# CODEJIN/Glow_TTS

Hardware: AMD Instinct MI355X
Metric: mel-frames/sec (train fwd+bwd) (higher is better)
Workload: dtype bf16; 1 GPU; BASELINE config 2: Vanilla single-speaker, LJSpeech-shaped synthetic (80-mel, 800 frames, 120 tokens), batch=32/GPU, fixed Set F, Train_Step = forward+losses+backward+clip_grad_norm+RAdam+Noam schedule; mode=Vanilla, global_batch=32, mel_frames=800, parallelism=dp1

## Files before the change

glow_tts_amd/abi.py:

```python
import ctypes
from ctypes import POINTER, c_char_p

ABI_VERSION = 7
OK, E_ARG, E_LAUNCH = 0, -1, -2
F32, BF16 = 0, 1
PERM_NONE, PERM_PAIR = 0, 1
APRO_NONE, APRO_PAIRMUL, APRO_SQNEG = 0, 1, 2
EPI_LINEAR, EPI_GATE, EPI_RESSKIP, EPI_COUPLE, EPI_DGATE = 0, 1, 2, 3, 4
F_BIAS, F_RELU, F_ADD_IN0, F_MASK, F_ACCUM, F_FIRST, F_LAST, F_REVERSE, F_COLMASK, F_DROPOUT = 1, 2, 4, 8, 16, 32, 64, 128, 256, 512
F_COND_ROWS, F_GATE_IN0, F_COND_FX = 1024, 2048, 4096
IO_A_BF16, IO_IN0_BF16, IO_OUT0_BF16 = 1, 2, 4
WIO_DY_BF16, WIO_X_BF16, WIO_WIDE, WIO_DMA = 1, 2, 4, 8
ROW_PAD = 2
MAX_WN_LAYERS = 8
WN_SLAB_BYTES = 24576
WN_FUSED_MAX_LAYERS = 4
PREP_MAX_JOBS = 22
WN_BWD_MAX_JOBS = 8
SUM_MAX_SEGS = 12
C2D_MAX_LAYERS = 8
SAMPLE_SCAN_CHUNK = 1024
SAMPLE_TILE = 64
GE2E_MAX_MEL, GE2E_MAX_H, GE2E_MAX_STACKS, GE2E_MAX_E = 512, 768, 8, 1024

I, L, F, U, P = ctypes.c_int, ctypes.c_int64, ctypes.c_float, ctypes.c_uint32, ctypes.c_void_p
PI, PL = POINTER(I), POINTER(L)


def _fields(*groups):
    return [(name, t) for names, t in groups for name in names.split()]


class Packed(ctypes.Structure):
    c_name = "glowtts_packed"
    _fields_ = _fields(("w", P), ("npad kchunks", I))


class FlowDims(ctypes.Structure):
    c_name = "glowtts_flow_dims"
    _fields_ = _fields(("B T C H L ksize precision", I), ("drop_p", F), ("seed", U), ("seed_ptr", P), ("act_bf16", I))


class FlowParams(ctypes.Structure):
    c_name = "glowtts_flow_params"
    _fields_ = _fields(("an_logs an_bias winfo", P),
                       ("start", Packed), ("in_ rs", Packed * MAX_WN_LAYERS), ("end", Packed),
                       ("start_t", Packed), ("in_t rs_t", Packed * MAX_WN_LAYERS), ("end_t", Packed),
                       ("b_start", P), ("b_in b_rs", P * MAX_WN_LAYERS), ("b_end", P),
                       ("cond", P), ("ldcond", L), ("cond_rows", I), ("wn_img wn_img_t", P))


class FlowActs(ctypes.Structure):
    c_name = "glowtts_flow_acts"
    _fields_ = _fields(("xin xmid xout", P), ("hs gates", P * MAX_WN_LAYERS), ("skip outs rowmask", P), ("acts", P * MAX_WN_LAYERS),
                       ("skip_bf xa_bf next_an_logs next_an_bias next_winfo next_xmid next_xout next_xa_bf", P), ("actnorm_done", I))


class FlowGrads(ctypes.Structure):
    c_name = "glowtts_flow_grads"
    _fields_ = _fields(("dx dlogdet douts dskip", P), ("dh dins", P * MAX_WN_LAYERS), ("defer_wgrad", I),
                       ("scratch d_an dw_start db_start", P), ("dw_in db_in dw_rs db_rs", P * MAX_WN_LAYERS),
                       ("dw_end db_end dcond douts_bf", P), ("coupling_done", I), ("prev_xmid prev_outs prev_douts prev_douts_bf pitch_rows", P),
                       ("pitch_ns dh0_bf16", I))


class WnBwdJob(ctypes.Structure):
    c_name = "glowtts_wn_bwd_job"
    _fields_ = _fields(("dw v g inv_norm dv dg", P), ("rows", L), ("cols reserved", I))


class SumSeg(ctypes.Structure):
    c_name = "glowtts_sum_seg"
    _fields_ = _fields(("dst", P), ("off n", L))


class WgradJob(ctypes.Structure):
    c_name = "glowtts_wgrad_job"
    _fields_ = _fields(("dy x xmask dw dbias", P), ("lddy ldx", L), ("m ca xpro perm perm_h tile0 mt nt rows reserved", I))


class PrepJob(ctypes.Structure):
    c_name = "glowtts_prep_job"
    _fields_ = _fields(("v g inv_out packed", P), ("outer_stride inner_stride w_stride g_stride", L),
                       ("batch inner O I taps transpose perm perm_h o_ext npad kchunks tiles block0 reserved", I),
                       ("twin", P), ("twin_outer twin_inner twin_half", L), ("twin_batch twin_npad", I))


class ConvArgs(ctypes.Structure):
    c_name = "glowtts_conv_args"
    _fields_ = _fields(("a", P), ("lda", L), ("a2", P), ("lda2", L), ("ca1 ca apro rows", I), ("w", P),
                       ("n npad kchunks taps pad precision epi flags h rows_per_utt", I), ("bias rowmask cond", P), ("ldcond", L),
                       ("out0", P), ("ld0", L), ("out1", P), ("ld1", L), ("in0", P), ("ldi0", L), ("batch", I),
                       ("a_bstride w_bstride bias_bstride out_bstride mask_bstride", L), ("ncols_valid", P),
                       ("seed", U), ("drop_p", F), ("seed_ptr", P), ("io_flags", I))


class WgradArgs(ctypes.Structure):
    c_name = "glowtts_wgrad_args"
    _fields_ = _fields(("dy", P), ("lddy", L), ("x", P), ("ldx", L), ("xpro", I), ("xmask", P),
                       ("rows m ca taps pad perm perm_h precision splits accumulate", I), ("dw dbias", P), ("io_flags", I))


class PackJob(ctypes.Structure):
    c_name = "glowtts_pack_job"
    _fields_ = _fields(("w packed", P), ("O I taps transpose perm perm_h N K npad kchunks block0 reserved", I))


class OptJob(ctypes.Structure):
    c_name = "glowtts_opt_job"
    _fields_ = _fields(("p g m v", P), ("n block0", L))


class C2dPackJob(ctypes.Structure):
    c_name = "glowtts_c2d_pack_job"
    _fields_ = _fields(("w img", P), ("Ci Co cls N K npad kchunks block0", I))


class C2dReduceJob(ctypes.Structure):
    c_name = "glowtts_c2d_reduce_job"
    _fields_ = _fields(("partial dw", P), ("splits Ci Co block0", I))


SIGNATURES = {
    "glowtts_abi_version": (I, []),
    "glowtts_device_arch": (I, [c_char_p, I]),
    "glowtts_launch_count": (L, [c_char_p]),
    "glowtts_launch_log_reset": (None, []),
    "glowtts_launch_log_dump": (I, [c_char_p, I]),
    "glowtts_mfma_clock_probe": (I, [P, I, I, PI, P]),
    "glowtts_debug_stamp": (I, [P, P]),
    "glowtts_step_seed": (I, [P] * 3),
    "glowtts_mas_dp_f32": (I, [P] * 5 + [I] * 3 + [F, P]),
    "glowtts_mas_dp_f32_t": (I, [P] * 5 + [I] * 3 + [F, P]),
    "glowtts_mas_path_from_idx": (I, [P, P] + [I] * 4 + [P]),
    "glowtts_mas_f32": (I, [P] * 5 + [I] * 3 + [F, P]),
    "glowtts_mas_f32_host": (I, [P] * 4 + [I] * 3 + [F, I]),
    "glowtts_pack_weight": (I, [P] + [I] * 7 + [P, PI, PI, P]),
    "glowtts_pack_job_init": (I, [POINTER(PackJob), P] + [I] * 7 + [P, I, PI, PL]),
    "glowtts_pack_weight_multi": (I, [P] + [I] * 3 + [P]),
    "glowtts_pack_weight_batched": (I, [P] + [I] * 8 + [P, PI, PI, P]),
    "glowtts_pack_weight_strided": (I, [P] + [I] * 9 + [P] + [L] * 3 + [P]),
    "glowtts_prep_jobs_twin_in": (I, [P, PI, PI]),
    "glowtts_prep_job_init": (I, [P] * 4 + [I] * 8 + [P] + [L] * 4 + [I, PI]),
    "glowtts_prep_launch": (I, [P] + [I] * 3 + [P]),
    "glowtts_prep_launch_dev": (I, [P] + [I] * 3 + [P]),
    "glowtts_conv_chain": (I, [P] * 3),
    "glowtts_conv_cl": (I, [P, P]),
    "glowtts_squeeze_rows": (I, [P] * 4 + [I] * 4 + [P]),
    "glowtts_unsqueeze_rows": (I, [P] * 3 + [I] * 5 + [F, P]),
    "glowtts_inv1x1_prepare": (I, [P, P, I, P]),
    "glowtts_actnorm_inv1x1": (I, [P] * 6 + [L, I, I, P]),
    "glowtts_actnorm_inv1x1_pass_bf": (I, [P] * 8 + [L, I, P]),
    "glowtts_actnorm_inv1x1_pass": (I, [P] * 7 + [L, I, P]),
    "glowtts_actnorm_stats": (I, [P] * 4 + [L, I, P]),
    "glowtts_actnorm_stats_scratch_floats": (L, [L, I]),
    "glowtts_actnorm_from_stats": (I, [P] * 3 + [I, P]),
    "glowtts_coupling_bwd": (I, [P] * 6 + [L] + [I] * 3 + [P]),
    "glowtts_coupling_bwd_bf16": (I, [P] * 7 + [L] + [I] * 3 + [P]),
    "glowtts_fill_zero": (I, [P, L, P]),
    "glowtts_actnorm_inv1x1_bwd": (I, [P] * 9 + [L, I, P]),
    "glowtts_actnorm_bwd_blocks": (L, [L]),
    "glowtts_actnorm_inv1x1_bwd_coupling": (I, [P] * 8 + [L, I] + [P] * 5 + [I, I, P]),
    "glowtts_colsum_batched": (I, [P, P] + [I] * 3 + [L, L, P]),
    "glowtts_decoder_param_grads": (I, [P] * 7 + [I] * 4 + [P]),
    "glowtts_decoder_logdet": (I, [P, L] + [P] * 5 + [I] * 5 + [P]),
    "glowtts_wgrad_cl": (I, [P, P]),
    "glowtts_wgrad_grouped": (I, [P] + [I] * 9 + [P]),
    "glowtts_wgrad_grouped_io": (I, [P] + [I] * 10 + [P]),
    "glowtts_wgrad_grouped_phased": (I, [P] + [I] * 5 + [P]),
    "glowtts_flow_forward": (I, [P] * 4),
    "glowtts_flow_inverse": (I, [P] * 4),
    "glowtts_flow_encode": (I, [P] * 4),
    "glowtts_flow_backward": (I, [P] * 5),
    "glowtts_wavenet_image_bytes": (I, [I, I, PL]),
    "glowtts_wavenet_pack_images": (I, [P] * 5 + [I] * 3 + [P] * 3),
    "glowtts_wavenet_prep_jobs": (I, [P, I, PI, PI] + [P] * 13 + [I] * 3 + [P, I, P]),
    "glowtts_wavenet_fwd": (I, [P] * 5 + [I, I, P]),
    "glowtts_wavenet_bwd": (I, [P] * 5),
    "glowtts_wavenet_debug_safe_waits": (None, [I]),
    "glowtts_utt_colsum": (I, [P, L, P, L] + [I] * 5 + [P]),
    "glowtts_cond_linear_fwd": (I, [P] * 6 + [I] * 4 + [P]),
    "glowtts_cond_linear_bwd_scratch_floats": (L, [I] * 3),
    "glowtts_cond_linear_supported": (I, [I] * 3),
    "glowtts_fx_to_float": (I, [P, P, L, P]),
    "glowtts_cond_linear_bwd": (I, [P, L] + [P] * 9 + [I] * 3 + [P]),
    "glowtts_gru_fwd": (I, [P] * 5 + [I] * 3 + [P]),
    "glowtts_gru_bwd": (I, [P] * 6 + [I] * 3 + [P]),
    "glowtts_gst_supported": (I, [I] * 7),
    "glowtts_gst_keep_floats": (L, [I] * 6),
    "glowtts_gst_fwd": (I, [P, P, I] + [P] * 13 + [I] * 7 + [P]),
    "glowtts_gst_bwd": (I, [P] * 3 + [I] + [P] * 18 + [I] * 7 + [P]),
    "glowtts_conv3x3s2_supported": (I, [I] * 5),
    "glowtts_conv3x3s2_image_bytes": (I, [I] * 3 + [PL, PL]),
    "glowtts_conv3x3s2_pack_job_init": (I, [POINTER(C2dPackJob), P] + [I] * 4 + [P, I, PI]),
    "glowtts_conv3x3s2_pack": (I, [P] + [I] * 3 + [P]),
    "glowtts_conv3x3s2_fwd": (I, [P] * 4 + [I] * 7 + [P]),
    "glowtts_conv3x3s2_dgrad": (I, [P, POINTER(P), P, P] + [I] * 6 + [P]),
    "glowtts_conv3x3s2_wgrad_scratch_floats": (L, [I] * 5),
    "glowtts_conv3x3s2_wgrad": (I, [P] * 3 + [I] * 6 + [PI, P]),
    "glowtts_conv3x3s2_wgrad_reduce": (I, [POINTER(C2dReduceJob), I, P]),
    "glowtts_layernorm_fwd": (I, [P] * 8 + [L, I, F, I, F, U, P, P]),
    "glowtts_layernorm_fwd_io": (I, [P] * 8 + [L, I, F, I, F, U] + [P] * 3),
    "glowtts_proj_layernorm": (I, [P, L, P, I] + [P] * 10 + [L, I, F, F, U, P, P]),
    "glowtts_layernorm_qkv": (I, [P] * 10 + [I, P, P, L, I, F, P]),
    "glowtts_layernorm_scratch_floats": (L, [L, I]),
    "glowtts_layernorm_bwd": (I, [P] * 9 + [L, I, I, F, P]),
    "glowtts_layernorm_bwd_io": (I, [P] * 9 + [L, I, I, F, P, P, F, P]),
    "glowtts_gate_bwd": (I, [P] * 4 + [L, I, F, P]),
    "glowtts_gate_bwd_io": (I, [P] * 4 + [L, I, F, I, P]),
    "glowtts_token_masks": (I, [P] * 3 + [I, I, P]),
    "glowtts_embedding_fwd": (I, [P] * 4 + [I] * 3 + [F, P]),
    "glowtts_embedding_bwd": (I, [P] * 4 + [I] * 4 + [F, P]),
    "glowtts_rpr_attention_fwd": (I, [P] * 6 + [I] * 5 + [F, U, P, P]),
    "glowtts_rpr_attention_scratch_floats": (L, [I] * 5),
    "glowtts_rpr_attention_bwd": (I, [P] * 11 + [I] * 5 + [F, U, P, P]),
    "glowtts_rpr_attention_fwd_prec": (I, [P] * 6 + [I] * 5 + [F, U, P, I, P]),
    "glowtts_rpr_attention_bwd_partial_rows": (L, [I] * 5),
    "glowtts_rpr_attention_fwd_eval": (I, [P] * 5 + [I] * 6 + [P]),
    "glowtts_rpr_attention_bwd_prec": (I, [P] * 11 + [I] * 5 + [F, U, P, I, P]),
    "glowtts_logprior_prep": (I, [P] * 9 + [I] * 5 + [PI, PI, P]),
    "glowtts_expand_fwd": (I, [P] * 3 + [I] * 4 + [P]),
    "glowtts_expand_bwd": (I, [P] * 3 + [I] * 4 + [P]),
    "glowtts_duration_targets": (I, [P] * 3 + [I] * 3 + [P]),
    "glowtts_mle_loss_fwd": (I, [P] * 8 + [L] + [I] * 3 + [P]),
    "glowtts_mle_loss_bwd": (I, [P] * 8 + [L, P, I, P]),
    "glowtts_expand_pair_targets": (I, [P] * 8 + [I] * 4 + [P]),
    "glowtts_prior_loss_bwd": (I, [P] * 10 + [I] * 4 + [P]),
    "glowtts_mse_loss_fwd": (I, [P] * 3 + [L, F, P, I] + [P] * 3),
    "glowtts_mse_loss_bwd": (I, [P] * 4 + [L, F, P, I, P, P]),
    "glowtts_prior_loss": (I, [P] * 17 + [I] * 6 + [P]),
    "glowtts_dur_proj_supported": (I, [I]),
    "glowtts_dur_proj_fwd": (I, [P] * 5 + [I] * 4 + [P]),
    "glowtts_dur_proj_bwd": (I, [P] * 9 + [I] * 4 + [P]),
    "glowtts_prior_split_fwd": (I, [P] * 3 + [I] * 4 + [P]),
    "glowtts_prior_split_bwd": (I, [P] * 3 + [I] * 4 + [P]),
    "glowtts_weightnorm_fwd": (I, [P] * 4 + [L, I, P]),
    "glowtts_weightnorm_bwd": (I, [P] * 6 + [L, I, P]),
    "glowtts_weightnorm_bwd_multi": (I, [P, I, P]),
    "glowtts_opt_chunk": (I, []),
    "glowtts_multi_grad_norm": (I, [P, I, I, F] + [P] * 3),
    "glowtts_sum_slices": (I, [P, P, I, L, P]),
    "glowtts_sum_slices_seg": (I, [P, I, L, P, I, P]),
    "glowtts_multi_grad_scale": (I, [P, I, I, P, P]),
    "glowtts_radam_step": (I, [P, I, I] + [P] * 3),
    "glowtts_vocoder_supported": (I, [I] * 3),
    "glowtts_mel_to_linear_f32": (I, [P] * 4 + [I] * 4 + [F, P]),
    "glowtts_stft_f32": (I, [P] * 5 + [I] * 6 + [P]),
    "glowtts_istft_f32": (I, [P] * 6 + [I] * 6 + [P]),
    "glowtts_overlap_add_f32": (I, [P] * 4 + [I] * 6 + [P]),
    "glowtts_griffin_lim_step_f32": (I, [P] * 6 + [F, P] + [I] * 6 + [P]),
    "glowtts_mel_analysis_f32": (I, [P] * 7 + [I] * 8 + [F] * 3 + [P]),
    "glowtts_yin_f32": (I, [P] * 4 + [I] * 7 + [F, F, P]),
    "glowtts_prior_sample": (I, [P] * 9 + [I] * 4 + [P]),
    "glowtts_pwg_supported": (I, [I] * 5),
    "glowtts_pwg_condition": (I, [P] * 5 + [I] + [P] * 2 + [I] * 4 + [P]),
    "glowtts_pwg_first": (I, [P] * 6 + [I] * 4 + [P]),
    "glowtts_pwg_layer": (I, [P] * 9 + [I] * 8 + [P]),
    "glowtts_pwg_head": (I, [P] * 7 + [I] * 4 + [F, P]),
    "glowtts_ge2e_supported": (I, [I] * 4),
    "glowtts_ge2e_image_floats": (L, [I] * 3),
    "glowtts_ge2e_work_floats": (L, [L] + [I] * 3),
    "glowtts_ge2e_pack": (I, [P] * 6 + [I] * 4 + [P]),
    "glowtts_ge2e_forward": (I, [P] * 9 + [I] * 7 + [P]),
    "glowtts_ge2e_train_image_floats": (L, [I] * 2),
    "glowtts_ge2e_train_keep_floats": (L, [L] + [I] * 3),
    "glowtts_ge2e_train_loss_work_floats": (L, [L] + [I] * 2),
    "glowtts_ge2e_train_work_floats": (L, [L] + [I] * 4),
    "glowtts_ge2e_train_pack": (I, [P] * 3 + [I] * 3 + [P]),
    "glowtts_ge2e_train_forward": (I, [P] * 7 + [I] * 6 + [P]),
    "glowtts_ge2e_train_loss": (I, [P] * 6 + [I] * 3 + [P]),
    "glowtts_ge2e_train_backward": (I, [P] * 8 + [I] * 5 + [P]),
    "glowtts_ge2e_train_wgrad": (I, [P] * 8 + [I] * 6 + [P]),
}
```

glow_tts_amd/csrc/actnorm_math.h:

```cpp
#pragma once
__device__ __forceinline__ void actnorm_mix4(const float (&x)[4], const float (&e)[4], const float (&b)[4], const float (&w)[16], float m, float (&o)[4])
{
    float v[4];
#pragma unroll
    for (int k = 0; k < 4; ++k) v[k] = __builtin_fmaf(e[k], x[k], b[k]) * m;
#pragma unroll
    for (int k = 0; k < 4; ++k)
        o[k] = __builtin_fmaf(w[k * 4 + 3], v[3], __builtin_fmaf(w[k * 4 + 2], v[2], __builtin_fmaf(w[k * 4 + 1], v[1], w[k * 4 + 0] * v[0]))) * m;
}
```

glow_tts_amd/csrc/flow.hip:

```cpp
#include <hip/hip_runtime.h>
#include <stdint.h>
#include <string.h>
#include <stdlib.h>
#include "../../include/glowtts_hip.h"
#include "tunable.h"

namespace {

#define CHECK(x) do { int rc_ = (x); if (rc_ != GLOWTTS_OK) return rc_; } while (0)

struct Ctx {
    const glowtts_flow_dims* d; const glowtts_flow_params* p; const glowtts_flow_acts* a; void* s;
    int Tp, R, C2, H, pad;
};

Ctx make_ctx(const glowtts_flow_dims* d, const glowtts_flow_params* p, const glowtts_flow_acts* a, void* s) {
    Ctx c{d, p, a, s, 0, 0, 0, 0, 0};
    c.Tp = d->T + 2 * GLOWTTS_ROW_PAD; c.R = d->B * c.Tp; c.C2 = d->C / 2; c.H = d->H; c.pad = (d->ksize - 1) / 2;
    return c;
}

int check_dims(const glowtts_flow_dims* d) {
    if (!d || d->B < 1 || d->T < 1 || d->C < 4 || (d->C & 3) || d->H < 1 || (d->H & 3) || d->L < 1 || d->L > GLOWTTS_MAX_WN_LAYERS) return GLOWTTS_E_ARG;
    if (d->ksize != 1 && d->ksize != 3 && d->ksize != 5) return GLOWTTS_E_ARG;
// ... 35 lines not shown
            a.out0 = g; a.ld0 = 2 * H; a.io_flags = bf ? (GLOWTTS_IO_A_BF16 | GLOWTTS_IO_OUT0_BF16) : 0;
            if (acts) { a.out1 = acts; a.ld1 = H; }
            CHECK(glowtts_conv_cl(&a, c.s));
        }
        const bool last = (l == L - 1);
        glowtts_conv_args rs = base_args(c, p->rs[l], 1);
        {
            glowtts_conv_args& a = rs;
            if (acts) { a.a = acts; a.lda = H; a.ca = H; }
            else      { a.a = g; a.lda = 2 * H; a.ca = H; a.apro = GLOWTTS_APRO_PAIRMUL; }
            a.n = last ? H : 2 * H; a.h = H;
            a.epi = GLOWTTS_EPI_RESSKIP; a.flags = (l == 0 ? GLOWTTS_F_FIRST : 0) | (last ? GLOWTTS_F_LAST : 0);
            a.bias = p->b_rs[l];
            a.in0 = hin; a.ldi0 = H; a.out0 = last ? A->skip : hout; a.ld0 = H; a.out1 = A->skip; a.ld1 = H;
            a.io_flags = bf ? (GLOWTTS_IO_A_BF16 | GLOWTTS_IO_IN0_BF16 | GLOWTTS_IO_OUT0_BF16) : 0;
            if (bf && last && A->skip_bf) { a.out0 = A->skip_bf; a.ld0 = H; }
        }
        if (!last) { CHECK(glowtts_conv_cl(&rs, c.s)); continue; }
        glowtts_conv_args a = base_args(c, p->end, 1);
        if (bf && A->skip_bf) { a.a = A->skip_bf; a.io_flags = GLOWTTS_IO_A_BF16; } else a.a = A->skip;
        a.lda = H; a.ca = H; a.n = c.d->C; a.h = c.C2;
        a.epi = GLOWTTS_EPI_COUPLE; a.flags = reverse ? GLOWTTS_F_REVERSE : 0; a.bias = p->b_end;
        a.in0 = xsrc + c.C2; a.ldi0 = c.d->C;
        a.out0 = xdst + c.C2; a.ld0 = c.d->C;
        a.out1 = keep ? A->outs : nullptr; a.ld1 = p->end.npad;
        const bool chain = GLOWTTS_TUNABLE("GLOWTTS_CHAIN", 1) != 0;
        if (chain && bf && acts && A->skip_bf && glowtts_conv_chain(&rs, &a, c.s) == GLOWTTS_OK) continue;
        CHECK(glowtts_conv_cl(&rs, c.s));
        CHECK(glowtts_conv_cl(&a, c.s));
    }
    return GLOWTTS_OK;
}

__global__ void copy_half_kernel(const float* __restrict__ src, float* __restrict__ dst, long rows, int C, int n)
{
    const int q = n / 4;
    const long total = rows * q;
    for (long i = blockIdx.x * 256L + threadIdx.x; i < total; i += (long)gridDim.x * 256) {
        const long r = i / q; const int c = (int)(i - r * q) * 4;
        *reinterpret_cast<float4*>(dst + r * C + c) = *reinterpret_cast<const float4*>(src + r * C + c);
    }
}
int copy_half(const float* src, float* dst, long rows, int C, int n, void* s) {
    if (src == dst) return GLOWTTS_OK;
    if (n & 3) return GLOWTTS_E_ARG;
    long g = (rows * (n / 4) + 255) / 256; if (g > 2048) g = 2048;
    hipLaunchKernelGGL(copy_half_kernel, dim3((int)g), dim3(256), 0, static_cast<hipStream_t>(s), src, dst, rows, C, n);
    return hipGetLastError() == hipSuccess ? GLOWTTS_OK : GLOWTTS_E_LAUNCH;
}

template <typename XT>
__global__ __launch_bounds__(256) void utt_colsum_kernel(const XT* __restrict__ x, long ldx, float* __restrict__ out, long ldout,
                                                         int rows_per_utt, int n, int perm, int perm_h)
{
    const int b = blockIdx.y;
    const int col = blockIdx.x * 256 + threadIdx.x;
    if (col >= n) return;
    int pc = col;
    if (perm == GLOWTTS_PERM_PAIR) { const int hs = col / perm_h, j = col - hs * perm_h; pc = (j >> 5) * 64 + hs * 32 + (j & 31); }
    const XT* xb = x + (long)b * rows_per_utt * ldx + pc;
    float s = 0.f;
    for (int r = 0; r < rows_per_utt; ++r) s += (float)xb[(long)r * ldx];
    out[(long)b * ldout + col] = s;
}

int utt_colsum(const float* x, int64_t ldx, float* out, int64_t ldout, int B, int rows_per_utt, int n, int perm, int perm_h, bool x_bf16, void* stream)
{
    if (!x || !out || B < 1 || rows_per_utt < 1 || n < 1) return GLOWTTS_E_ARG;
    const dim3 grid((n + 255) / 256, B);
    hipStream_t s = static_cast<hipStream_t>(stream);
    if (x_bf16) hipLaunchKernelGGL(utt_colsum_kernel<__bf16>, grid, dim3(256), 0, s, reinterpret_cast<const __bf16*>(x), (long)ldx, out, (long)ldout, rows_per_utt, n, perm, perm_h);
    else hipLaunchKernelGGL(utt_colsum_kernel<float>, grid, dim3(256), 0, s, x, (long)ldx, out, (long)ldout, rows_per_utt, n, perm, perm_h);
    return hipGetLastError() == hipSuccess ? GLOWTTS_OK : GLOWTTS_E_LAUNCH;
}

}

extern "C" int glowtts_utt_colsum(const float* x, int64_t ldx, float* out, int64_t ldout, int B, int rows_per_utt, int n,
                                  int perm, int perm_h, void* stream)
{
    return utt_colsum(x, ldx, out, ldout, B, rows_per_utt, n, perm, perm_h, false, stream);
}

extern "C" int glowtts_flow_forward(const glowtts_flow_dims* d, const glowtts_flow_params* p, const glowtts_flow_acts* a, void* stream)
{
    CHECK(check_dims(d));
    if (!p || !a || !a->xin || !a->xmid || !a->xout || !a->rowmask || !a->outs) return GLOWTTS_E_ARG;
    if (!a->skip && !(p->wn_img && a->skip_bf)) return GLOWTTS_E_ARG;
    if (d->act_bf16) for (int l = 0; l < d->L; ++l) if (!a->acts[l]) return GLOWTTS_E_ARG;
    const Ctx c = make_ctx(d, p, a, stream);
    if (a->next_xmid && (!p->wn_img || !a->next_an_logs || !a->next_an_bias || !a->next_winfo || !a->next_xout)) return GLOWTTS_E_ARG;
    if (!a->actnorm_done)
        CHECK(glowtts_actnorm_inv1x1_pass_bf(a->xin, a->xmid, a->xout, a->xa_bf, p->an_logs, p->an_bias, p->winfo, a->rowmask, c.R, d->C, stream));
    return coupling_net(c, a->xmid, a->xout, false, true);
}

extern "C" int glowtts_flow_encode(const glowtts_flow_dims* d, const glowtts_flow_params* p, const glowtts_flow_acts* a, void* stream)
{
    CHECK(check_dims(d));
    if (d->drop_p != 0.f) return GLOWTTS_E_ARG;
    if (!p || !a || !a->xin || !a->xmid || !a->xout || !a->rowmask) return GLOWTTS_E_ARG;
    if (!p->wn_img) {
        if (!a->skip || !a->hs[0] || !a->hs[1] || !a->gates[0]) return GLOWTTS_E_ARG;
        if (d->act_bf16 && !a->acts[0]) return GLOWTTS_E_ARG;
    }
    if (a->next_xmid) {
        if (!p->wn_img || !a->next_an_logs || !a->next_an_bias || !a->next_winfo || !a->next_xout) return GLOWTTS_E_ARG;
        if (a->next_xmid == a->xmid || a->next_xout == a->xmid || a->xout == a->xmid || a->next_xmid == a->xout) return GLOWTTS_E_ARG;
    }
    const Ctx c = make_ctx(d, p, a, stream);
    if (!a->actnorm_done)
        CHECK(glowtts_actnorm_inv1x1_pass_bf(a->xin, a->xmid, a->xout, a->xa_bf, p->an_logs, p->an_bias, p->winfo, a->rowmask, c.R, d->C, stream));
    return coupling_net(c, a->xmid, a->xout, false, false);
}

extern "C" int glowtts_flow_inverse(const glowtts_flow_dims* d, const glowtts_flow_params* p, const glowtts_flow_acts* a, void* stream)
{
    CHECK(check_dims(d));
    if (!p || !a || !a->xin || !a->xmid || !a->xout || !a->rowmask) return GLOWTTS_E_ARG;
    if (!p->wn_img) {
        if (!a->skip || !a->hs[0] || !a->hs[1] || !a->gates[0]) return GLOWTTS_E_ARG;
        if (d->act_bf16 && !a->acts[0]) return GLOWTTS_E_ARG;
    }
    const Ctx c = make_ctx(d, p, a, stream);
    CHECK(copy_half(a->xout, a->xmid, c.R, d->C, c.C2, stream));
    CHECK(coupling_net(c, a->xout, a->xmid, true, false));
    return glowtts_actnorm_inv1x1(a->xmid, a->xin, p->an_logs, p->an_bias, p->winfo, a->rowmask, c.R, d->C, 1, stream);
}

extern "C" int glowtts_flow_backward(const glowtts_flow_dims* d, const glowtts_flow_params* p, const glowtts_flow_acts* a,
                                     const glowtts_flow_grads* g, void* stream)
{
    CHECK(check_dims(d));
    if (!p || !a || !g || !g->dx || !g->dlogdet || !g->dskip || !g->dh[0] || !g->dins[0] || !g->scratch) return GLOWTTS_E_ARG;
    const Ctx c = make_ctx(d, p, a, stream);
    const int H = c.H, L = d->L, C = d->C, C2 = c.C2, R = c.R;
    const int ldo = p->end.npad;
    const int ldin = p->in[0].npad;
    auto wargs = [&](const float* dy, int lddy, int m, const float* x, int ldx, int ca, int taps, float* dw, float* db) {
        glowtts_wgrad_args w; memset(&w, 0, sizeof(w));
        w.dy = dy; w.lddy = lddy; w.m = m; w.x = x; w.ldx = ldx; w.ca = ca; w.rows = R; w.taps = taps; w.pad = (taps - 1) / 2;
        w.precision = d->precision; w.splits = 0; w.accumulate = 1; w.dw = dw; w.dbias = db;
        return w;
    };

    const bool bf = d->act_bf16 != 0;
    const bool bfg = bf;
    const bool dbf = bfg && g->douts_bf != nullptr;
    if (!g->douts && (!dbf || !g->defer_wgrad)) return GLOWTTS_E_ARG;
    if (g->coupling_done) {  }
    else if (dbf) CHECK(glowtts_coupling_bwd_bf16(g->dx, a->xmid, a->outs, g->douts, g->douts_bf, a->rowmask, g->dlogdet, R, C, ldo, c.Tp, stream));
    else     CHECK(glowtts_coupling_bwd(g->dx, a->xmid, a->outs, g->douts, a->rowmask, g->dlogdet, R, C, ldo, c.Tp, stream));
    if (p->wn_img_t) {
        CHECK(glowtts_wavenet_bwd(d, p, a, g, stream));
        if (g->prev_outs && g->d_an) return GLOWTTS_E_ARG;
        if (g->prev_outs)
            return glowtts_actnorm_inv1x1_bwd_coupling(g->dx, g->dx, a->xin, p->an_logs, p->an_bias, p->winfo, a->rowmask, g->scratch, R, C,
                                                       g->prev_xmid, g->prev_outs, g->prev_douts, g->prev_douts_bf, g->dlogdet, ldo, c.Tp, stream);
        return glowtts_actnorm_inv1x1_bwd(g->dx, g->dx, a->xin, p->an_logs, p->an_bias, p->winfo, a->rowmask, g->d_an, g->scratch, R, C, stream);
    }
    glowtts_conv_args endq = base_args(c, p->end_t, 1);
    endq.a = dbf ? g->douts_bf : g->douts; endq.lda = ldo; endq.ca = ldo; endq.n = H; endq.epi = GLOWTTS_EPI_LINEAR; endq.flags = GLOWTTS_F_MASK;
    endq.out0 = g->dskip; endq.ld0 = H; endq.io_flags = (dbf ? GLOWTTS_IO_A_BF16 : 0) | (bfg ? GLOWTTS_IO_OUT0_BF16 : 0);
    bool end_done = false;
    if (!g->defer_wgrad) {
        glowtts_wgrad_args w = wargs(g->douts, ldo, ldo, a->skip, H, H, 1, g->dw_end, g->db_end);
        w.perm = GLOWTTS_PERM_PAIR; w.perm_h = C2;
        CHECK(glowtts_wgrad_cl(&w, stream));
    }
    const bool wg = !g->defer_wgrad;
    for (int l = L - 1; l >= 0; --l) {
        const bool last = (l == L - 1);
        float* dnext = last ? nullptr : g->dh[l + 1];
        float* dthis = g->dh[l];
        float* dins = g->dins[l];
        {
            glowtts_conv_args q = base_args(c, p->rs_t[l], 1);
            if (last) { q.a = g->dskip; q.lda = H; q.ca = H; }
            else      { q.a = dnext; q.lda = H; q.ca1 = H; q.a2 = g->dskip; q.lda2 = H; q.ca = 2 * H; }
            q.n = H; q.epi = GLOWTTS_EPI_DGATE; q.in0 = a->gates[l]; q.ldi0 = 2 * H; q.out0 = dins; q.ld0 = ldin;
            q.drop_p = d->drop_p; q.seed = d->seed + (uint32_t)l; q.seed_ptr = d->seed_ptr;
            q.io_flags = bf ? (GLOWTTS_IO_IN0_BF16 | GLOWTTS_IO_OUT0_BF16 | (bfg ? GLOWTTS_IO_A_BF16 : 0)) : 0;
            if (g->dcond && p->cond) {
                q.out1 = reinterpret_cast<float*>(g->dcond + (int64_t)l * 2 * H); q.ld1 = p->ldcond; q.flags |= GLOWTTS_F_COND_FX;
                if (g->pitch_rows) {
                    if (g->pitch_ns < 1 || g->pitch_ns > 2) return GLOWTTS_E_ARG;
                    q.cond = g->pitch_rows; q.ldcond = g->pitch_ns; q.flags |= GLOWTTS_F_COND_ROWS;
                }
            }
            if (last) {
                const bool chain = GLOWTTS_TUNABLE("GLOWTTS_CHAIN", 1) != 0 && GLOWTTS_TUNABLE("GLOWTTS_CHAIN_BWD", 1) != 0;
                if (!(chain && dbf && glowtts_conv_chain(&endq, &q, stream) == GLOWTTS_OK)) {
                    CHECK(glowtts_conv_cl(&endq, stream));
                    CHECK(glowtts_conv_cl(&q, stream));
                }
                end_done = true;
            } else {
                CHECK(glowtts_conv_cl(&q, stream));
            }
        }
        if (wg) {
            if (last) {
                glowtts_wgrad_args w = bf ? wargs(g->dskip, H, H, a->acts[l], H, H, 1, g->dw_rs[l], g->db_rs[l])
                                          : wargs(g->dskip, H, H, a->gates[l], 2 * H, H, 1, g->dw_rs[l], g->db_rs[l]);
                w.xpro = bf ? GLOWTTS_APRO_NONE : GLOWTTS_APRO_PAIRMUL; w.io_flags = bf ? (GLOWTTS_WIO_X_BF16 | (bfg ? GLOWTTS_WIO_DY_BF16 : 0)) : 0;
                CHECK(glowtts_wgrad_cl(&w, stream));
            } else {
                glowtts_wgrad_args w = bf ? wargs(dnext, H, H, a->acts[l], H, H, 1, g->dw_rs[l], g->db_rs[l])
                                          : wargs(dnext, H, H, a->gates[l], 2 * H, H, 1, g->dw_rs[l], g->db_rs[l]);
                w.xpro = bf ? GLOWTTS_APRO_NONE : GLOWTTS_APRO_PAIRMUL; w.io_flags = bf ? (GLOWTTS_WIO_X_BF16 | (bfg ? GLOWTTS_WIO_DY_BF16 : 0)) : 0;
                CHECK(glowtts_wgrad_cl(&w, stream));
                glowtts_wgrad_args w2 = bf ? wargs(g->dskip, H, H, a->acts[l], H, H, 1, g->dw_rs[l] + (int64_t)H * H, g->db_rs[l] + H)
                                           : wargs(g->dskip, H, H, a->gates[l], 2 * H, H, 1, g->dw_rs[l] + (int64_t)H * H, g->db_rs[l] + H);
                w2.xpro = bf ? GLOWTTS_APRO_NONE : GLOWTTS_APRO_PAIRMUL; w2.io_flags = bf ? (GLOWTTS_WIO_X_BF16 | (bfg ? GLOWTTS_WIO_DY_BF16 : 0)) : 0;
                CHECK(glowtts_wgrad_cl(&w2, stream));
            }
        }
        {
            glowtts_conv_args q = base_args(c, p->in_t[l], d->ksize);
            q.a = dins; q.lda = ldin; q.ca = ldin; q.n = H; q.epi = GLOWTTS_EPI_LINEAR;
            q.flags = GLOWTTS_F_MASK | (last ? 0 : GLOWTTS_F_ADD_IN0);
            q.in0 = last ? nullptr : dnext; q.ldi0 = H; q.out0 = dthis; q.ld0 = H;
            q.io_flags = bf ? (GLOWTTS_IO_A_BF16 | (bfg && !last ? GLOWTTS_IO_IN0_BF16 : 0) | (bfg && (l > 0 || g->dh0_bf16) ? GLOWTTS_IO_OUT0_BF16 : 0)) : 0;
            CHECK(glowtts_conv_cl(&q, stream));
        }
        if (wg) {
            glowtts_wgrad_args w = wargs(dins, ldin, ldin, a->hs[l], H, H, d->ksize, g->dw_in[l], g->db_in[l]);
            w.perm = GLOWTTS_PERM_PAIR; w.perm_h = H; w.io_flags = bf ? (GLOWTTS_WIO_DY_BF16 | GLOWTTS_WIO_X_BF16) : 0;
            CHECK(glowtts_wgrad_cl(&w, stream));
        }
    }
    if (!end_done) return GLOWTTS_E_ARG;
    float* dh0 = g->dh[0];
    {
        glowtts_conv_args q = base_args(c, p->start_t, 1);
        const bool h0bf = bfg && g->dh0_bf16;
        q.a = dh0; q.lda = H; q.ca = H; q.n = C2; q.epi = GLOWTTS_EPI_LINEAR; q.flags = GLOWTTS_F_ACCUM;
        q.out0 = g->dx; q.ld0 = C; q.io_flags = h0bf ? GLOWTTS_IO_A_BF16 : 0;
        CHECK(glowtts_conv_cl(&q, stream));
        if (wg) {
            if (h0bf && !a->xa_bf) return GLOWTTS_E_ARG;
            glowtts_wgrad_args w = h0bf ? wargs(dh0, H, H, reinterpret_cast<const float*>(a->xa_bf), C2, C2, 1, g->dw_start, g->db_start)
                                        : wargs(dh0, H, H, a->xmid, C, C2, 1, g->dw_start, g->db_start);
            if (h0bf) w.io_flags = GLOWTTS_WIO_DY_BF16 | GLOWTTS_WIO_X_BF16;
            CHECK(glowtts_wgrad_cl(&w, stream));
        }
    }
    if (g->prev_outs && g->d_an) return GLOWTTS_E_ARG;
    if (g->prev_outs)
        return glowtts_actnorm_inv1x1_bwd_coupling(g->dx, g->dx, a->xin, p->an_logs, p->an_bias, p->winfo, a->rowmask, g->scratch, R, C,
                                                   g->prev_xmid, g->prev_outs, g->prev_douts, g->prev_douts_bf, g->dlogdet, ldo, c.Tp, stream);
    return glowtts_actnorm_inv1x1_bwd(g->dx, g->dx, a->xin, p->an_logs, p->an_bias, p->winfo, a->rowmask, g->d_an, g->scratch, R, C, stream);
}
```

glow_tts_amd/csrc/flow_ops.hip:

```cpp
#include <hip/hip_runtime.h>
#include <stdint.h>
#include <stdlib.h>
#include "../../include/glowtts_hip.h"
#include "launch_log.h"
#include "tunable.h"
#include "actnorm_math.h"

namespace {

#define PADR GLOWTTS_ROW_PAD

#ifndef GLOWTTS_SQ_TS
#define GLOWTTS_SQ_TS 16
#endif
constexpr int SQ_TS = GLOWTTS_SQ_TS;
template <bool TO_ROWS>
__global__ __launch_bounds__(256) void squeeze_kernel(float* __restrict__ mel, float* __restrict__ rows,
                                                      float* __restrict__ rowmask, const int64_t* __restrict__ lengths,
                                                      int Cm, int Tm, int T, int ns, float fill, int use_fill)
{
    extern __shared__ float tile[];
    const int b = blockIdx.y;
    const int t0 = blockIdx.x * SQ_TS;
    const int Tp = T + 2 * PADR;
// ... 181 lines not shown
        const float dm = d * m, dl = (d * e * xb + dld[r / rows_per_utt]) * m;
        if (douts) {
            douts[r * ldo + pc] = dm;
            douts[r * ldo + pc + 32] = dl;
        }
        if (douts16) { douts16[r * ldo + pc] = (__bf16)dm; douts16[r * ldo + pc + 32] = (__bf16)dl; }
        dz[r * C + C2 + j] = d * e * m;
    }
}
__global__ void zero_kernel(float* __restrict__ p, long n)
{
    for (long i = blockIdx.x * 256L + threadIdx.x; i < n; i += (long)gridDim.x * 256) p[i] = 0.f;
}

struct NextCoupling {
    const float* xmid; const float* outs; float* douts; __bf16* douts16; const float* dld; int ldo; int rows_per_utt;
};

__global__ __launch_bounds__(256) void actnorm_inv_bwd_kernel(const float* __restrict__ dz, float* __restrict__ dx,
                                                              const float* __restrict__ x, const float* __restrict__ logs,
                                                              const float* __restrict__ bias, const float* __restrict__ winfo,
                                                              const float* __restrict__ rowmask, float* __restrict__ partial,
                                                              long rows, int C, int rows_per_block, const NextCoupling nc)
{
    const int G = C / 4, C2 = C / 2;
    extern __shared__ float red[];
    float w[16];
#pragma unroll
    for (int i = 0; i < 16; ++i) w[i] = winfo[i];
    const long r0 = (long)blockIdx.x * rows_per_block;
    const long r1 = min(rows, r0 + rows_per_block);
    const int tpg = 256 / G;
    const int g = threadIdx.x % G;
    const int rl = threadIdx.x / G;
    float accW[16], accL[4], accB[4];
#pragma unroll
    for (int i = 0; i < 16; ++i) accW[i] = 0.f;
#pragma unroll
    for (int i = 0; i < 4; ++i) { accL[i] = 0.f; accB[i] = 0.f; }
    const int ch[4] = {2 * g, 2 * g + 1, C2 + 2 * g, C2 + 2 * g + 1};
    float el[4], bs[4];
#pragma unroll
    for (int k = 0; k < 4; ++k) { el[k] = expf(logs[ch[k]]); bs[k] = bias[ch[k]]; }
    if (rl < tpg) {
        for (long r = r0 + rl; r < r1; r += tpg) {
            const float m = rowmask[r];
            const float2 dlo = *reinterpret_cast<const float2*>(dz + r * C + 2 * g);
            const float2 dhi = *reinterpret_cast<const float2*>(dz + r * C + C2 + 2 * g);
            const float2 xlo = *reinterpret_cast<const float2*>(x + r * C + 2 * g);
            const float2 xhi = *reinterpret_cast<const float2*>(x + r * C + C2 + 2 * g);
            const float d[4] = {dlo.x * m, dlo.y * m, dhi.x * m, dhi.y * m};
            const float xv[4] = {xlo.x, xlo.y, xhi.x, xhi.y};
            float y[4], dy[4], o[4];
#pragma unroll
            for (int k = 0; k < 4; ++k) y[k] = (bs[k] + el[k] * xv[k]) * m;
#pragma unroll
            for (int k = 0; k < 4; ++k) dy[k] = (w[0 * 4 + k] * d[0] + w[1 * 4 + k] * d[1] + w[2 * 4 + k] * d[2] + w[3 * 4 + k] * d[3]) * m;
#pragma unroll
            for (int a = 0; a < 4; ++a)
#pragma unroll
                for (int k = 0; k < 4; ++k) accW[a * 4 + k] += d[a] * y[k];
#pragma unroll
            for (int k = 0; k < 4; ++k) { o[k] = dy[k] * el[k]; accL[k] += o[k] * xv[k]; accB[k] += dy[k]; }
            *reinterpret_cast<float2*>(dx + r * C + 2 * g) = make_float2(o[0], o[1]);
            if (nc.outs) {
                const float dl = nc.dld[r / nc.rows_per_utt];
                const float2 xb = *reinterpret_cast<const float2*>(nc.xmid + r * C + C2 + 2 * g);
                float ob[2];
#pragma unroll
                for (int k = 0; k < 2; ++k) {
                    const int j = 2 * g + k, pc = (j >> 5) * 64 + (j & 31);
                    const float d = o[2 + k], e = expf(nc.outs[r * nc.ldo + pc + 32]);
                    const float dm = d * m, dlg = (d * e * (k ? xb.y : xb.x) + dl) * m;
                    if (nc.douts) { nc.douts[r * nc.ldo + pc] = dm; nc.douts[r * nc.ldo + pc + 32] = dlg; }
                    if (nc.douts16) { nc.douts16[r * nc.ldo + pc] = (__bf16)dm; nc.douts16[r * nc.ldo + pc + 32] = (__bf16)dlg; }
                    ob[k] = d * e * m;
                    for (int jp = C2 + j; jp < nc.ldo / 2; jp += C2) {
                        const int pp = (jp >> 5) * 64 + (jp & 31);
                        if (nc.douts) { nc.douts[r * nc.ldo + pp] = 0.f; nc.douts[r * nc.ldo + pp + 32] = 0.f; }
                        if (nc.douts16) { nc.douts16[r * nc.ldo + pp] = (__bf16)0.f; nc.douts16[r * nc.ldo + pp + 32] = (__bf16)0.f; }
                    }
                }
                *reinterpret_cast<float2*>(dx + r * C + C2 + 2 * g) = make_float2(ob[0], ob[1]);
            } else {
                *reinterpret_cast<float2*>(dx + r * C + C2 + 2 * g) = make_float2(o[2], o[3]);
            }
        }
    }
    float* out = partial + (long)blockIdx.x * (2 * C + 16);
    for (int q = 0; q < 24; ++q) {
        float v = (q < 16) ? accW[q] : (q < 20 ? accL[q - 16] : accB[q - 20]);
        red[q * 256 + threadIdx.x] = (rl < tpg) ? v : 0.f;
    }
    __syncthreads();
    {
        const int q = threadIdx.x >> 4, part = threadIdx.x & 15;
        float s = 0.f;
#pragma unroll
        for (int t = 0; t < 16; ++t) s += red[q * 256 + t * 16 + part];
#pragma unroll
        for (int o = 8; o >= 1; o >>= 1) s += __shfl_xor(s, o, 16);
        if (part == 0) out[2 * C + q] = s;
    }
    for (int i = threadIdx.x; i < 2 * 4 * G; i += 256) {
        const int which = i / (4 * G), k = (i / G) % 4, gg = i % G;
        float s = 0.f;
        for (int t = gg; t < tpg * G; t += G) s += red[(16 + which * 4 + k) * 256 + t];
        const int c = (k < 2) ? (2 * gg + k) : (C2 + 2 * gg + (k - 2));
        out[which * C + c] = s;
    }
}

__global__ __launch_bounds__(256) void actnorm_inv_bwd4_kernel(const float* __restrict__ dz, float* __restrict__ dx,
                                                               const float* __restrict__ x, const float* __restrict__ logs,
                                                               const float* __restrict__ bias, const float* __restrict__ winfo,
                                                               const float* __restrict__ rowmask, float* __restrict__ partial,
                                                               long rows, int C, int rows_per_block, const NextCoupling nc)
{
    const int Q = C / 8, C2 = C / 2;
    extern __shared__ float red[];
    float w[16];
#pragma unroll
    for (int i = 0; i < 16; ++i) w[i] = winfo[i];
    const long r0 = (long)blockIdx.x * rows_per_block;
    const long r1 = min(rows, r0 + rows_per_block);
    const int tpq = 256 / Q;
    const int q = threadIdx.x % Q, rl = threadIdx.x / Q;
    float accW[16], accL[8], accB[8];
#pragma unroll
    for (int i = 0; i < 16; ++i) accW[i] = 0.f;
#pragma unroll
    for (int i = 0; i < 8; ++i) { accL[i] = 0.f; accB[i] = 0.f; }
    float el[8], bs[8];
    {
        const float4 la = *reinterpret_cast<const float4*>(logs + 4 * q), lb = *reinterpret_cast<const float4*>(logs + C2 + 4 * q);
        const float4 ba = *reinterpret_cast<const float4*>(bias + 4 * q), bb = *reinterpret_cast<const float4*>(bias + C2 + 4 * q);
        const float lv[8] = {la.x, la.y, la.z, la.w, lb.x, lb.y, lb.z, lb.w}, bv[8] = {ba.x, ba.y, ba.z, ba.w, bb.x, bb.y, bb.z, bb.w};
#pragma unroll
        for (int k = 0; k < 8; ++k) { el[k] = expf(lv[k]); bs[k] = bv[k]; }
    }
    if (rl < tpq) {
        for (long r = r0 + rl; r < r1; r += tpq) {
            const float m = rowmask[r];
            const float4 dlo = *reinterpret_cast<const float4*>(dz + r * C + 4 * q), dhi = *reinterpret_cast<const float4*>(dz + r * C + C2 + 4 * q);
            const float4 xlo = *reinterpret_cast<const float4*>(x + r * C + 4 * q), xhi = *reinterpret_cast<const float4*>(x + r * C + C2 + 4 * q);
            float4 lg = make_float4(0.f, 0.f, 0.f, 0.f), xb = lg;
            float dl = 0.f;
            const int j0 = 4 * q, pc = (j0 >> 5) * 64 + (j0 & 31);
            if (nc.outs) {
                lg = *reinterpret_cast<const float4*>(nc.outs + r * nc.ldo + pc + 32);
                xb = *reinterpret_cast<const float4*>(nc.xmid + r * C + C2 + 4 * q);
                dl = nc.dld[r / nc.rows_per_utt];
            }
            const float dv[8] = {dlo.x * m, dlo.y * m, dlo.z * m, dlo.w * m, dhi.x * m, dhi.y * m, dhi.z * m, dhi.w * m};
            const float xv[8] = {xlo.x, xlo.y, xlo.z, xlo.w, xhi.x, xhi.y, xhi.z, xhi.w};
            float o[8];
#pragma unroll
            for (int e = 0; e < 2; ++e) {
                const int sl[4] = {2 * e, 2 * e + 1, 4 + 2 * e, 5 + 2 * e};
                float y[4], dy[4];
#pragma unroll
                for (int k = 0; k < 4; ++k) y[k] = (bs[sl[k]] + el[sl[k]] * xv[sl[k]]) * m;
#pragma unroll
                for (int k = 0; k < 4; ++k)
                    dy[k] = (w[0 * 4 + k] * dv[sl[0]] + w[1 * 4 + k] * dv[sl[1]] + w[2 * 4 + k] * dv[sl[2]] + w[3 * 4 + k] * dv[sl[3]]) * m;
#pragma unroll
                for (int a = 0; a < 4; ++a)
#pragma unroll
                    for (int k = 0; k < 4; ++k) accW[a * 4 + k] += dv[sl[a]] * y[k];
#pragma unroll
                for (int k = 0; k < 4; ++k) { o[sl[k]] = dy[k] * el[sl[k]]; accL[sl[k]] += o[sl[k]] * xv[sl[k]]; accB[sl[k]] += dy[k]; }
            }
            *reinterpret_cast<float4*>(dx + r * C + 4 * q) = make_float4(o[0], o[1], o[2], o[3]);
            if (nc.outs) {
                const float lgv[4] = {lg.x, lg.y, lg.z, lg.w}, xbv[4] = {xb.x, xb.y, xb.z, xb.w};
                float dm[4], dg[4], ob[4];
#pragma unroll
                for (int k = 0; k < 4; ++k) {
                    const float d = o[4 + k], e = expf(lgv[k]);
                    dm[k] = d * m; dg[k] = (d * e * xbv[k] + dl) * m; ob[k] = d * e * m;
                }
                float* dob = nc.douts ? nc.douts + r * nc.ldo : nullptr;
                if (dob) {
                    *reinterpret_cast<float4*>(dob + pc) = make_float4(dm[0], dm[1], dm[2], dm[3]);
                    *reinterpret_cast<float4*>(dob + pc + 32) = make_float4(dg[0], dg[1], dg[2], dg[3]);
                }
                typedef __bf16 bf4 __attribute__((ext_vector_type(4)));
                if (nc.douts16) {
                    bf4 a, b;
#pragma unroll
                    for (int k = 0; k < 4; ++k) { a[k] = (__bf16)dm[k]; b[k] = (__bf16)dg[k]; }
                    *reinterpret_cast<bf4*>(nc.douts16 + r * nc.ldo + pc) = a;
                    *reinterpret_cast<bf4*>(nc.douts16 + r * nc.ldo + pc + 32) = b;
                }
                for (int jp = C2 + j0; jp < nc.ldo / 2; jp += C2) {
                    const int pp = (jp >> 5) * 64 + (jp & 31);
                    if (dob) {
                        *reinterpret_cast<float4*>(dob + pp) = make_float4(0.f, 0.f, 0.f, 0.f);
                        *reinterpret_cast<float4*>(dob + pp + 32) = make_float4(0.f, 0.f, 0.f, 0.f);
                    }
                    if (nc.douts16) {
                        *reinterpret_cast<uint2*>(nc.douts16 + r * nc.ldo + pp) = make_uint2(0u, 0u);
                        *reinterpret_cast<uint2*>(nc.douts16 + r * nc.ldo + pp + 32) = make_uint2(0u, 0u);
                    }
                }
                *reinterpret_cast<float4*>(dx + r * C + C2 + 4 * q) = make_float4(ob[0], ob[1], ob[2], ob[3]);
            } else {
                *reinterpret_cast<float4*>(dx + r * C + C2 + 4 * q) = make_float4(o[4], o[5], o[6], o[7]);
            }
        }
    }
    float* out = partial + (long)blockIdx.x * (2 * C + 16);
    for (int i = 0; i < 32; ++i) {
        const float v = (i < 16) ? accW[i] : (i < 24 ? accL[i - 16] : accB[i - 24]);
        red[i * 256 + threadIdx.x] = (rl < tpq) ? v : 0.f;
    }
    __syncthreads();
    {
        const int e = threadIdx.x >> 4, part = threadIdx.x & 15;
        float s = 0.f;
#pragma unroll
        for (int t = 0; t < 16; ++t) s += red[e * 256 + t * 16 + part];
#pragma unroll
        for (int o = 8; o >= 1; o >>= 1) s += __shfl_xor(s, o, 16);
        if (part == 0) out[2 * C + e] = s;
    }
    for (int i = threadIdx.x; i < 2 * 8 * Q; i += 256) {
        const int which = i / (8 * Q), sl = (i / Q) % 8, qq = i % Q;
        float s = 0.f;
        for (int t = qq; t < tpq * Q; t += Q) s += red[(16 + which * 8 + sl) * 256 + t];
        const int c = (sl < 4) ? (4 * qq + sl) : (C2 + 4 * qq + (sl - 4));
        out[which * C + c] = s;
    }
}

__global__ __launch_bounds__(1024) void logdet_partial_kernel(const float* __restrict__ outs_all, long flow_stride,
                                                              const float* __restrict__ logs_all, const float* __restrict__ winfo_all,
                                                              const float* __restrict__ rowmask, float* __restrict__ part,
                                                              int B, int Tp, int C, int ldo)
{
    __shared__ float red[3][16];
    const int f = blockIdx.x, b = blockIdx.y;
    const int C2 = C / 2, wave = threadIdx.x >> 6, lane = threadIdx.x & 63;
    const float* outs = outs_all + (long)f * flow_stride + (long)b * Tp * ldo;
    const float* rm = rowmask + (long)b * Tp;
    float s = 0.f, len = 0.f, ls = 0.f;
    for (int t0 = wave; t0 < Tp; t0 += 64) {
        float m[4], v[4][2];
#pragma unroll
        for (int u = 0; u < 4; ++u) {
            const int t = t0 + 16 * u;
            const bool in = t < Tp;
            m[u] = in ? rm[t] : 0.f;
#pragma unroll
            for (int h = 0; h < 2; ++h) {
                const int j = lane + 64 * h;
                v[u][h] = (in && j < C2) ? outs[(long)t * ldo + (j >> 5) * 64 + 32 + (j & 31)] : 0.f;
            }
        }
#pragma unroll
        for (int u = 0; u < 4; ++u) { len += m[u]; s += (v[u][0] + v[u][1]) * m[u]; }
    }
    for (int j = lane + 128; j < C2; j += 64)
        for (int t = wave; t < Tp; t += 16) s += outs[(long)t * ldo + (j >> 5) * 64 + 32 + (j & 31)] * rm[t];
    for (int c = threadIdx.x; c < C; c += 1024) ls += logs_all[f * C + c];
#pragma unroll
    for (int o = 32; o >= 1; o >>= 1) { s += __shfl_xor(s, o); ls += __shfl_xor(ls, o); }
    if (lane == 0) { red[0][wave] = s; red[1][wave] = len; red[2][wave] = ls; }
    __syncthreads();
    if (threadIdx.x == 0) {
        float S = 0.f, L = 0.f, A = 0.f;
        for (int w = 0; w < 16; ++w) { S += red[0][w]; L += red[1][w]; A += red[2][w]; }
        part[f * B + b] = S + (A + winfo_all[f * 36 + 32] * (float)(C / 4)) * L;
    }
}
__global__ void logdet_final_kernel(const float* __restrict__ part, float* __restrict__ logdet, int F, int B)
{
    const int b = blockIdx.x * blockDim.x + threadIdx.x;
    if (b >= B) return;
    float s = 0.f;
    for (int f = 0; f < F; ++f) s += part[f * B + b];
    logdet[b] = s;
}

inline int grid_for(long total, int per = 256, int cap = 2048) { long g = (total + per - 1) / per; return (int)(g > cap ? cap : (g < 1 ? 1 : g)); }
#define RET_LAUNCH() return hipGetLastError() == hipSuccess ? GLOWTTS_OK : GLOWTTS_E_LAUNCH

}

extern "C" int glowtts_squeeze_rows(const float* mel, float* rows, float* rowmask, const int64_t* lengths,
                                    int B, int Cm, int Tm, int ns, void* stream)
{
    if (!mel || !rows || !lengths || B < 1 || Cm < 1 || ns < 1 || Tm < ns) return GLOWTTS_E_ARG;
    const int T = Tm / ns;
    const size_t lds = (size_t)Cm * (SQ_TS * ns + 1) * sizeof(float);
    hipLaunchKernelGGL(squeeze_kernel<true>, dim3((T + SQ_TS - 1) / SQ_TS, B), dim3(256), lds, static_cast<hipStream_t>(stream),
                       const_cast<float*>(mel), rows, rowmask, lengths, Cm, Tm, T, ns, 0.f, 0);
    RET_LAUNCH();
}

extern "C" int glowtts_unsqueeze_rows(const float* rows, float* mel, const int64_t* lengths,
                                      int B, int Cm, int Tm, int ns, int use_fill, float fill, void* stream)
{
    if (!mel || !rows || !lengths || B < 1 || Cm < 1 || ns < 1 || Tm < ns) return GLOWTTS_E_ARG;
    const int T = Tm / ns;
    const size_t lds = (size_t)Cm * (SQ_TS * ns + 1) * sizeof(float);
    hipLaunchKernelGGL(squeeze_kernel<false>, dim3((T + SQ_TS - 1) / SQ_TS, B), dim3(256), lds, static_cast<hipStream_t>(stream),
                       mel, const_cast<float*>(rows), (float*)nullptr, lengths, Cm, Tm, T, ns, fill, use_fill);
    RET_LAUNCH();
}

extern "C" int glowtts_inv1x1_prepare(const float* W, float* winfo, int F, void* stream)
{
    if (!W || !winfo || F < 1) return GLOWTTS_E_ARG;
    hipLaunchKernelGGL(inv4x4_kernel, dim3((F + 63) / 64), dim3(64), 0, static_cast<hipStream_t>(stream), W, winfo, F);
    RET_LAUNCH();
}

extern "C" int glowtts_actnorm_inv1x1(const float* xin, float* xout, const float* logs, const float* bias,
                                      const float* winfo, const float* rowmask, int64_t rows, int C, int reverse, void* stream)
{
    if (!xin || !xout || !logs || !bias || !winfo || !rowmask || rows < 1 || C < 4 || (C & 3)) return GLOWTTS_E_ARG;
    hipStream_t s = static_cast<hipStream_t>(stream);
    const int grid = grid_for(rows * (C / 4));
    if (reverse) hipLaunchKernelGGL(actnorm_inv_kernel<true>, dim3(grid), dim3(256), 0, s, xin, xout, logs, bias, winfo, rowmask, (long)rows, C, (float*)nullptr);
    else         hipLaunchKernelGGL(actnorm_inv_kernel<false>, dim3(grid), dim3(256), 0, s, xin, xout, logs, bias, winfo, rowmask, (long)rows, C, (float*)nullptr);
    RET_LAUNCH();
}

extern "C" int glowtts_actnorm_inv1x1_pass(const float* xin, float* xout, float* xpass, const float* logs, const float* bias, const float* winfo,
                                           const float* rowmask, int64_t rows, int C, void* stream)
{
    if (!xin || !xout || !xpass || !logs || !bias || !winfo || !rowmask || rows < 1 || C < 4 || (C & 3)) return GLOWTTS_E_ARG;
    hipLaunchKernelGGL(actnorm_inv_kernel<false>, dim3(grid_for(rows * (C / 4))), dim3(256), 0, static_cast<hipStream_t>(stream),
                       xin, xout, logs, bias, winfo, rowmask, (long)rows, C, xpass == xout ? (float*)nullptr : xpass);
    RET_LAUNCH();
}

extern "C" int glowtts_actnorm_inv1x1_pass_bf(const float* xin, float* xout, float* xpass, void* xa_bf, const float* logs, const float* bias, const float* winfo,
                                              const float* rowmask, int64_t rows, int C, void* stream)
{
    if (!xin || !xout || !logs || !bias || !winfo || !rowmask || rows < 1 || C < 4 || (C & 3)) return GLOWTTS_E_ARG;
    GLOWTTS_NOTE_STATIC("actnorm_inv1x1_pass%s", "");
    hipLaunchKernelGGL(actnorm_inv_kernel<false>, dim3(grid_for(rows * (C / 4))), dim3(256), 0, static_cast<hipStream_t>(stream),
                       xin, xout, logs, bias, winfo, rowmask, (long)rows, C, (xpass == xout || !xpass) ? (float*)nullptr : xpass, static_cast<uint32_t*>(xa_bf));
    RET_LAUNCH();
}

extern "C" int glowtts_actnorm_stats(const float* x, const float* rowmask, float* stats, float* scratch,
                                     int64_t rows, int C, void* stream)
{
    if (!x || !rowmask || !stats || !scratch || rows < 1 || C < 1) return GLOWTTS_E_ARG;
    hipStream_t s = static_cast<hipStream_t>(stream);
    const int rpb = 64;
    const int nblk = (int)((rows + rpb - 1) / rpb);
    hipLaunchKernelGGL(colstats_partial_kernel, dim3(nblk), dim3(256), 0, s, x, rowmask, scratch, (long)rows, C, rpb);
    const int n = 2 * C + 1;
    hipLaunchKernelGGL(colstats_final_kernel, dim3((n + 3) / 4), dim3(256), 0, s, scratch, stats, nblk, n, 0L, 0L);
    RET_LAUNCH();
}

static bool an_bwd_wide(int C, const float* dz, const float* dx, const float* x, int ldo)
// ... 163 lines not shown
```

glow_tts_amd/csrc/wavenet_fused_bwd.hip:

```cpp
#include <hip/hip_runtime.h>
#include <stdint.h>
#include <string.h>
#include "../../include/glowtts_hip.h"
#include "tunable.h"
#include "launch_log.h"
#include "wavenet_common.h"

int glowtts_wavenet_safe_waits_flag();

namespace {

constexpr int BW_NS = 3;
constexpr int BOFF_DX = 0;
constexpr int BSZ_DX = WN_KCH * WN_WIN * 64;
constexpr int BOFF_DS = BOFF_DX + BSZ_DX;
constexpr int BSZ_T = WN_KCH * WN_XR * 64;
constexpr int BOFF_DT = BOFF_DS + BSZ_T;
constexpr int BOFF_RING = BOFF_DT + BSZ_T;
constexpr int BOFF_MK = BOFF_RING + BW_NS * WN_SLAB;
constexpr int BOFF_UT = BOFF_MK + WN_XR * 4;
constexpr int BOFF_P3 = BOFF_UT + WN_XR * 4;
constexpr int BW_LDS = BOFF_P3 + WN_KCH * 4 * 64;
static_assert(BW_LDS <= 160 * 1024, "LDS budget");
static_assert(BSZ_T >= WN_NW * 8 * 256, "the partial-sum exchange (8 registers per wave and round) reuses the gate-gradient tile");

struct wn_bwd_args {
    int rows, rows_per_utt, L, C2;
    const unsigned char* wimg;
    const void* douts_bf; int64_t ldo;
    const float* rowmask;
    const void* gates[WN_MAXL];
    float drop_p; uint32_t seed; const uint32_t* seed_ptr;
    void* dskip;
    void* dins[WN_MAXL]; int64_t ldin;
    void* dh[WN_MAXL];
    int dh0_bf16;
    float* dx; int64_t lddx;
    float* dcond; int64_t ldcond;
    long long* tl;
    int stagger;
};

template <bool DROP, bool COND, int ABL = 0>
__global__ __launch_bounds__(WN_NT) void wn_bwd_kernel(const wn_bwd_args p)
{
    extern __shared__ __attribute__((aligned(1024))) unsigned char wb_smem[];
    unsigned char* const DX = wb_smem + BOFF_DX;
    unsigned char* const DS = wb_smem + BOFF_DS;
    unsigned char* const DT = wb_smem + BOFF_DT;
    float* const MK = reinterpret_cast<float*>(wb_smem + BOFF_MK);
    int* const UT = reinterpret_cast<int*>(wb_smem + BOFF_UT);

    const int tid = threadIdx.x, lane = tid & 63;
    const int wave = __builtin_amdgcn_readfirstlane(tid >> 6);
    const int l15 = lane & 15, lq = lane >> 4;
    const int rf = wave >= 6 ? 1 : 0, cf = wave - rf * 6;
    const int cp = cf >> 1, kh = cf & 1;
    const int L = p.L;
    const int halo = WN_PAD * (L - 1);
    const int nvalid = WN_WIN - 2 * halo;
    const int v0 = blockIdx.x * nvalid;
    const int t0 = v0 - halo;
    const int xr0 = t0 - WN_PAD;
    const int lim = (p.rows - v0) < nvalid ? (p.rows - v0) : nvalid;
    const int jch0 = cf * 32 + l15;

    const int lrow = lane >> 2, qa = (lane & 3) ^ (((lane >> 4) & 1) << 1);
    const unsigned char* const wsrc = p.wimg + (uint32_t)((wave * 32 + lrow) * 64 + qa * 16);
    auto issue = [&](int s) __attribute__((always_inline)) {
        const unsigned char* src = wsrc + (size_t)s * WN_SLAB;
        unsigned char* dst = wb_smem + BOFF_RING + (s % BW_NS) * WN_SLAB + wave * 2048;
        __builtin_amdgcn_global_load_lds((const void __attribute__((address_space(1)))*)src, (void __attribute__((address_space(3)))*)dst, 16, 0, 0);
        __builtin_amdgcn_global_load_lds((const void __attribute__((address_space(1)))*)(src + 1024), (void __attribute__((address_space(3)))*)(dst + 1024), 16, 0, 0);
    };
    int snext = 0;
    int tli = 0;
    auto TLS = [&]() __attribute__((always_inline)) { if constexpr ((ABL & 64) != 0) { if (tid == 0) p.tl[blockIdx.x * 64 + tli] = (long long)__builtin_readcyclecounter(); ++tli; } };
    TLS();
    constexpr bool EXACT = !COND && !(ABL & 128);
    auto begin_step = [&](auto X_) __attribute__((always_inline)) -> const unsigned char* {
        constexpr int X = EXACT ? decltype(X_)::value : 0;
        asm volatile("s_waitcnt vmcnt(%0) lgkmcnt(0)\n\ts_barrier" :: "n"(2 + X) : "memory");
        return wb_smem + BOFF_RING + (snext % BW_NS) * WN_SLAB;
    };
    constexpr int XC = 2;
    auto end_step = [&]() __attribute__((always_inline)) {
        if (!(ABL & 1)) issue(snext + BW_NS - 1);
        ++snext;
    };
    auto plain_barrier = [&]() __attribute__((always_inline)) { asm volatile("s_waitcnt lgkmcnt(0)\n\ts_barrier" ::: "memory"); };

    issue(0); issue(1);
#ifdef GLOWTTS_TOOLS
    for (int k = 0; k < (int)((blockIdx.x >> 3) & 7) * p.stagger; ++k) __builtin_amdgcn_s_sleep(8);
#endif
    {
        const int per_row = (WN_H * 2) / 16;
#pragma unroll
        for (int k = 0; k < 3; ++k) {
            const int idx = tid + k * WN_NT;
            if (idx < WN_XR * per_row) {
                const int i = idx / per_row, pc = idx - i * per_row;
                int g = xr0 + i;
                g = g < 0 ? 0 : (g >= p.rows ? p.rows - 1 : g);
                const Chunk16 v = *reinterpret_cast<const Chunk16*>(static_cast<const unsigned char*>(p.douts_bf) + ((int64_t)g * p.ldo) * 2 + pc * 16);
                *reinterpret_cast<Chunk16*>(DT + (pc >> 2) * (WN_XR * 64) + swz16(i, pc & 3)) = v;
            }
        }
        if (tid < WN_XR) {
            int g = xr0 + tid;
            g = g < 0 ? 0 : (g >= p.rows ? p.rows - 1 : g);
            MK[tid] = p.rowmask[g];
            if (COND) UT[tid] = g / p.rows_per_utt;
        }
    }
    const int bl = swz16(l15, lq);
    const int offA = rf * 2048;
    const int rbw = rf * 32 + 4 * lq;
    auto tile_off_of = [](int l15x, int lqx, int h, int cy) __attribute__((always_inline)) -> int {
        return ((((2 * h + (l15x >> 3)) ^ (((lqx + cy) & 1) << 1)) & 3) << 4) + (l15x & 7) * 2;
    };
    auto fresh_lane = [&]() __attribute__((always_inline)) -> int { int a = lane; asm volatile("" : "+v"(a)); return a; };

    auto copy_out = [&](const unsigned char* tile, int trows, int row_off, void* dst, int row_bytes, int chunk_bytes, int off) __attribute__((always_inline)) {
        if constexpr ((ABL & 4) != 0) return;
        const Rsrc rd = mk_rsrc(dst, (long)p.rows * row_bytes);
        int tid_ = tid;
        asm volatile("" : "+v"(tid_));
#pragma unroll
        for (int k = 0; k < 2; ++k) {
            const int idx = tid_ + k * WN_NT;
            const int r = idx / 24, pc = idx - r * 24;
            const bool ok = r < lim;
            const Chunk16 v = lds16(tile + (pc >> 2) * (trows * 64) + swz16(row_off + (ok ? r : 0), pc & 3));
            __builtin_amdgcn_raw_buffer_store_b128(v, rd, ok ? (uint32_t)((v0 + r) * row_bytes + off + (pc >> 2) * chunk_bytes + (pc & 3) * 16) : OOB, 0, 0);
        }
    };

    f32x4 acc[2][4];
    f32x4 a3[2];
    auto zero_acc = [&]() __attribute__((always_inline)) {
#pragma unroll
        for (int rt = 0; rt < 2; ++rt)
#pragma unroll
            for (int ct = 0; ct < 4; ++ct) acc[rt][ct] = f32x4{0.f, 0.f, 0.f, 0.f};
        a3[0] = a3[1] = f32x4{0.f, 0.f, 0.f, 0.f};
    };
    auto mma192 = [&](const unsigned char* slot, const unsigned char* a0, const unsigned char* a1, bool third, int shift) __attribute__((always_inline)) {
        Chunk16 fa[2][2], fb[2][2], f3[2];
        int ar0 = offA + bl, ar1 = offA + 1024 + bl;
        if (shift) {
            const int ln = fresh_lane();
            ar0 = swz16(rf * 32 + (ln & 15) + shift, ln >> 4);
            ar1 = swz16(rf * 32 + 16 + (ln & 15) + shift, ln >> 4);
        }
#pragma unroll
        for (int c = 0; c < 2; ++c) {
            const unsigned char* At = c ? a1 : a0;
            fa[c][0] = lds16(At + ar0);
            fa[c][1] = lds16(At + ar1);
#pragma unroll
            for (int ct = 0; ct < 2; ++ct) fb[c][ct] = lds16(slot + c * 12288 + cf * 2048 + ct * 1024 + bl);
            if (third) f3[c] = lds16(At + 4096 + bl);
        }
        __builtin_amdgcn_sched_barrier(0);
#pragma unroll
        for (int c = 0; c < 2; ++c) {
#pragma unroll
            for (int ct = 0; ct < 2; ++ct)
#pragma unroll
                for (int rt = 0; rt < 2; ++rt) acc[rt][ct] = mfma16_bf16<!(ABL & 2)>(fa[c][rt], fb[c][ct], acc[rt][ct]);
            if (third) {
#pragma unroll
                for (int ct = 0; ct < 2; ++ct) a3[ct] = mfma16_bf16<!(ABL & 2)>(f3[c], fb[c][ct], a3[ct]);
            }
        }
        __builtin_amdgcn_sched_barrier(0);
    };
    const bool w3 = wave < 6;

    TLS();
    zero_acc();
#pragma unroll 1
    for (int j = 0; j < 3; ++j) {
        const unsigned char* slot = begin_step(IC<0>{});
        mma192(slot, DT + (2 * j) * (WN_XR * 64), DT + (2 * j + 1) * (WN_XR * 64), w3, 0);
        end_step();
    }
    TLS();
    {
        const int ln = fresh_lane(), l15x = ln & 15, lqx = ln >> 4;
// ... 170 lines not shown
            unsigned char* const dc = DT + cf * (WN_XR * 64) + (rb + roff) * 64;
#pragma unroll
            for (int h = 0; h < 2; ++h) {
                const int to0 = tile_off_of(l15x, lqx, h, 0), to1 = tile_off_of(l15x, lqx, h, 1);
#pragma unroll
                for (int rt = 0; rt < 2; ++rt)
#pragma unroll
                    for (int i2 = 0; i2 < 2; ++i2) {
                        const uint32_t w = pkd[rt][h][i2];
                        const int to = ((2 * i2 + roff) >> 2) ? to1 : to0;
                        *reinterpret_cast<unsigned short*>(dc + (16 * rt + 2 * i2) * 64 + to) = (unsigned short)(w & 0xFFFFu);
                        *reinterpret_cast<unsigned short*>(dc + (16 * rt + 2 * i2 + 1) * 64 + to) = (unsigned short)(w >> 16);
                    }
                if constexpr (last) {
                    if (w3 && lqx == 0) {
#pragma unroll
                        for (int i = 0; i < 4; ++i)
                            *reinterpret_cast<unsigned short*>(DT + cf * (WN_XR * 64) + (64 + i) * 64 + to0) = *reinterpret_cast<const unsigned short*>(wb_smem + BOFF_P3 + cf * 256 + i * 64 + to0);
                    }
                }
            }
        };

        zero_acc();
        {
            Chunk16 fa[2][2], fb[2][4];
            auto mma = [&](auto SET_) __attribute__((always_inline)) {
                constexpr int st = decltype(SET_)::value;
#pragma unroll
                for (int ct = 0; ct < 4; ++ct)
#pragma unroll
                    for (int rt = 0; rt < 2; ++rt) acc[rt][ct] = mfma16_bf16<!(ABL & 2)>(fa[st][rt], fb[st][ct], acc[rt][ct]);
            };
            const int lnI = fresh_lane(), l15i = lnI & 15, lqi = lnI >> 4;
            const uint32_t dtk = lds0 + (uint32_t)(BOFF_DT + kh * (WN_XR * 64));
            const uint32_t sbk = (uint32_t)(kh * 12288 + cp * 4096 + swz16(l15i, lqi));
            uint32_t ao0 = 0, ao1 = 0;
            auto step = [&](auto N_) __attribute__((always_inline)) {
                constexpr int n = decltype(N_)::value;
                constexpr int m = n >= 15 ? n - 15 : n, t = m / 3, jj = m - 3 * t, st = n & 1;
                const unsigned char* slot = begin_step(IC<((n == 1 || n == 16) && !(ABL & 4) ? XC : 0)>{});
                if constexpr (n == 0) copy_out(DT, WN_XR, halo + WN_PAD, pick4(p.dins, l), (int)p.ldin * 2, 128, 0);
                if constexpr (n == 15) TLS();
                if constexpr (n == 15) {
                    write_ds_half();
                    plain_barrier();
                    copy_out(DT, WN_XR, halo + WN_PAD, pick4(p.dins, l), (int)p.ldin * 2, 128, 64);
                }
                if constexpr (jj == 0) {
                    ao0 = dtk + (uint32_t)swz16(rf * 32 + l15i + t, lqi);
                    ao1 = dtk + (uint32_t)swz16(rf * 32 + 16 + l15i + t, lqi);
                }
                const uint32_t sa = lds_addr(slot) + sbk;
                fa[st][0] = lds16_asm<2 * jj * (WN_XR * 64)>(ao0);
                fa[st][1] = lds16_asm<2 * jj * (WN_XR * 64)>(ao1);
                fb[st][0] = lds16_asm<0>(sa); fb[st][1] = lds16_asm<1024>(sa); fb[st][2] = lds16_asm<2048>(sa); fb[st][3] = lds16_asm<3072>(sa);
                if constexpr (n > 0) { lgkm_wait<6>(fa[st ^ 1], fb[st ^ 1]); mma(IC<st ^ 1>{}); }
                __builtin_amdgcn_sched_barrier(0);
                end_step();
            };
            StaticForN<30>::run([&](auto J_) __attribute__((always_inline)) { step(J_); });
            lgkm_wait<0>(fa[1], fb[1]);
            mma(IC<1>{});
        }
        TLS();
        f32x4 fin[2][2];
        {
            const int lane = fresh_lane();
            float* const xs0 = reinterpret_cast<float*>(DT);
            float* const xs1 = reinterpret_cast<float*>(wb_smem + BOFF_RING + ((snext + BW_NS - 1) % BW_NS) * WN_SLAB);
            if constexpr (!(ABL & 16)) {
                plain_barrier();
#pragma unroll
                for (int h = 0; h < 2; ++h)
#pragma unroll
                    for (int i = 0; i < 4; ++i) {
                        xs0[(wave * 8 + h * 4 + i) * 64 + lane] = kh ? acc[0][h][i] : acc[0][2 + h][i];
                        xs1[(wave * 8 + h * 4 + i) * 64 + lane] = kh ? acc[1][h][i] : acc[1][2 + h][i];
                    }
                plain_barrier();
            }
#pragma unroll
            for (int h = 0; h < 2; ++h)
#pragma unroll
                for (int i = 0; i < 4; ++i) {
                    const float o0 = (ABL & 16) ? 0.f : xs0[((wave ^ 1) * 8 + h * 4 + i) * 64 + lane];
                    const float o1 = (ABL & 16) ? 0.f : xs1[((wave ^ 1) * 8 + h * 4 + i) * 64 + lane];
                    fin[0][h][i] = (kh ? acc[0][2 + h][i] : acc[0][h][i]) + o0;
                    fin[1][h][i] = (kh ? acc[1][2 + h][i] : acc[1][h][i]) + o1;
                }
        }
        TLS();
        {
            const int ln = fresh_lane(), l15x = ln & 15, lqx = ln >> 4;
            const int rb = rf * 32 + 4 * lqx;
            const int jch0 = cf * 32 + l15x;
            unsigned char* const xc = DX + cf * (WN_WIN * 64) + rb * 64;
            const float* const mk = MK + rb + WN_PAD;
            const bool fp32_rows = l == 0 && !p.dh0_bf16;
            const Rsrc r0 = mk_rsrc(p.dh[0], fp32_rows ? (long)p.rows * (WN_H * 4) : 0);
            const uint32_t own0 = (uint32_t)(rb - halo);
#pragma unroll
            for (int h = 0; h < 2; ++h) {
                const int to = tile_off_of(l15x, lqx, h, 0);
                const uint32_t v00 = (uint32_t)((t0 + rb) * (WN_H * 4) + (jch0 + 16 * h) * 4);
#pragma unroll
                for (int rt = 0; rt < 2; ++rt)
#pragma unroll
                    for (int i = 0; i < 4; ++i) {
                        const int c = 16 * rt + i;
                        unsigned short* xp = reinterpret_cast<unsigned short*>(xc + c * 64 + to);
                        const float xin = last ? 0.f : __uint_as_float((uint32_t)*xp << 16);
                        const float v = (fin[rt][h][i] + xin) * mk[c];
                        *xp = bf16_bits(v);
                        const bool ok = own0 + (uint32_t)c < (uint32_t)lim;
                        if constexpr (!(ABL & 4)) { if (fp32_rows) __builtin_amdgcn_raw_buffer_store_b32(__float_as_uint(v), r0, ok ? v00 + (uint32_t)(c * (WN_H * 4)) : OOB, 0, 0); }
                    }
            }
        }
    };
#pragma unroll 1
    for (int l = L - 1; l >= 0; --l) {
        if (l == L - 1) layer(IC<1>{}, l); else layer(IC<0>{}, l);
    }

    TLS();
    zero_acc();
#pragma unroll
    for (int j = 0; j < 2; ++j) {
        if (j == 0) asm volatile("s_waitcnt vmcnt(2) lgkmcnt(0)\n\ts_barrier" ::: "memory");
        else        asm volatile("s_waitcnt vmcnt(0) lgkmcnt(0)\n\ts_barrier" ::: "memory");
        const unsigned char* slot = wb_smem + BOFF_RING + (snext % BW_NS) * WN_SLAB;
        ++snext;
        if (j == 0 && p.dh0_bf16) copy_out(DX, WN_WIN, halo, p.dh[0], WN_H * 2, 64, 0);
        if (cf < 3) {
            Chunk16 fa[3][2], fb[3][2];
#pragma unroll
            for (int c = 0; c < 3; ++c) {
#pragma unroll
                for (int rt = 0; rt < 2; ++rt) fa[c][rt] = lds16(DX + (3 * j + c) * (WN_WIN * 64) + offA + rt * 1024 + bl);
#pragma unroll
                for (int ct = 0; ct < 2; ++ct) fb[c][ct] = lds16(slot + c * 8192 + cf * 2048 + ct * 1024 + bl);
            }
            __builtin_amdgcn_sched_barrier(0);
#pragma unroll
            for (int c = 0; c < 3; ++c)
#pragma unroll
                for (int ct = 0; ct < 2; ++ct)
#pragma unroll
                    for (int rt = 0; rt < 2; ++rt) acc[rt][ct] = mfma16_bf16<!(ABL & 2)>(fa[c][rt], fb[c][ct], acc[rt][ct]);
        }
    }
    TLS();
    if (cf < 3) {
        int rb = rbw;
        asm volatile("" : "+v"(rb));
        const Rsrc rx = mk_rsrc(p.dx, (long)p.rows * p.lddx * 4);
        const uint32_t own0 = (uint32_t)(rb - halo);
        float old[2][2][4];
#pragma unroll
        for (int h = 0; h < 2; ++h) {
            const bool cok = jch0 + 16 * h < p.C2;
            const uint32_t vx0 = (uint32_t)((t0 + rb) * (int)p.lddx + jch0 + 16 * h) * 4u;
#pragma unroll
            for (int rt = 0; rt < 2; ++rt)
#pragma unroll
                for (int i = 0; i < 4; ++i) {
                    const int c = 16 * rt + i;
                    const bool ok = cok && own0 + (uint32_t)c < (uint32_t)lim;
                    old[h][rt][i] = __uint_as_float(__builtin_amdgcn_raw_buffer_load_b32(rx, ok ? vx0 + (uint32_t)(c * (int)p.lddx * 4) : OOB, 0, 0));
                }
        }
#pragma unroll
        for (int h = 0; h < 2; ++h) {
            const bool cok = jch0 + 16 * h < p.C2;
            const uint32_t vx0 = (uint32_t)((t0 + rb) * (int)p.lddx + jch0 + 16 * h) * 4u;
#pragma unroll
            for (int rt = 0; rt < 2; ++rt)
#pragma unroll
                for (int i = 0; i < 4; ++i) {
                    const int c = 16 * rt + i;
                    const bool ok = cok && own0 + (uint32_t)c < (uint32_t)lim;
                    if constexpr (!(ABL & 4)) __builtin_amdgcn_raw_buffer_store_b32(__float_as_uint(old[h][rt][i] + acc[rt][h][i]), rx, ok ? vx0 + (uint32_t)(c * (int)p.lddx * 4) : OOB, 0, 0);
                }
        }
    }
    TLS();
}

template <bool DROP, bool COND, int ABL = 0>
int launch_wn_bwd(const wn_bwd_args& k, dim3 grid, hipStream_t s)
{
#ifdef GLOWTTS_TOOLS
    if constexpr (ABL == 0 && DROP && !COND) {
        switch (GLOWTTS_TUNABLE("GLOWTTS_WN_BWD_ABL", 0)) {
            case 1: return launch_wn_bwd<DROP, COND, 1>(k, grid, s);
            case 2: return launch_wn_bwd<DROP, COND, 2>(k, grid, s);
            case 3: return launch_wn_bwd<DROP, COND, 3>(k, grid, s);
            case 4: return launch_wn_bwd<DROP, COND, 4>(k, grid, s);
            case 8: return launch_wn_bwd<DROP, COND, 8>(k, grid, s);
            case 12: return launch_wn_bwd<DROP, COND, 12>(k, grid, s);
            case 13: return launch_wn_bwd<DROP, COND, 13>(k, grid, s);
            case 14: return launch_wn_bwd<DROP, COND, 14>(k, grid, s);
            case 16: return launch_wn_bwd<DROP, COND, 16>(k, grid, s);
            case 64: return launch_wn_bwd<DROP, COND, 64>(k, grid, s);
            case 29: return launch_wn_bwd<DROP, COND, 29>(k, grid, s);
            case 31: return launch_wn_bwd<DROP, COND, 31>(k, grid, s);
            default: break;
        }
    }
#endif
    if constexpr (ABL == 0 && DROP && !COND) {
        if (glowtts_wavenet_safe_waits_flag()) return launch_wn_bwd<DROP, COND, 128>(k, grid, s);
    }
    static bool attr_done = false;
    if (!attr_done) {
        if (hipFuncSetAttribute(reinterpret_cast<const void*>(&wn_bwd_kernel<DROP, COND, ABL>), hipFuncAttributeMaxDynamicSharedMemorySize, 160 * 1024) != hipSuccess) return GLOWTTS_E_LAUNCH;
        attr_done = true;
    }
    GLOWTTS_NOTE_STATIC("wn_bwd<%s%s>", DROP ? "drop" : "nodrop", COND ? ",cond" : "");
    hipLaunchKernelGGL((wn_bwd_kernel<DROP, COND, ABL>), grid, dim3(WN_NT), BW_LDS, s, k);
    return hipGetLastError() == hipSuccess ? GLOWTTS_OK : GLOWTTS_E_LAUNCH;
}

}

int glowtts_wavenet_pack_bwd_images(const float* w_start, const float* w_in, const float* w_rs, const float* w_rs_last, const float* w_end,
                                    int F, int L, int C2, void* img_bwd, void* stream)
{
    const int H = WN_H;
    const int64_t S = WN_SLAB, stride = (int64_t)(36 * L + 2) * S;
    unsigned char* img = static_cast<unsigned char*>(img_bwd);
    int rc = glowtts_pack_weight_strided(w_end, F, 1, 2 * C2, H, 1, 1, GLOWTTS_PERM_PAIR, C2, GLOWTTS_BF16, img, stride, 0, 0, stream);
    if (rc == GLOWTTS_OK) rc = glowtts_pack_weight_strided(w_rs_last, F, 1, H, H, 1, 1, GLOWTTS_PERM_NONE, 0, GLOWTTS_BF16, img + 3 * S, stride, 0, 0, stream);
    if (rc == GLOWTTS_OK && L > 1)
        rc = glowtts_pack_weight_strided(w_rs, F * (L - 1), L - 1, 2 * H, H, 1, 1, GLOWTTS_PERM_NONE, 0, GLOWTTS_BF16, img + (36 + 36 * (int64_t)(L - 2)) * S, stride, -36 * S, 0, stream);
    for (int half = 0; half < 2 && rc == GLOWTTS_OK; ++half)
        rc = glowtts_pack_weight_strided(w_in + (int64_t)half * H * H * WN_TAPS, F * L, L, H, H, WN_TAPS, 1, GLOWTTS_PERM_NONE, 0, GLOWTTS_BF16,
                                         img + (42 + 36 * (int64_t)(L - 2) + 15 * half) * S, stride, -36 * S, (int64_t)2 * H * H * WN_TAPS, stream);
    if (rc == GLOWTTS_OK) rc = glowtts_pack_weight_strided(w_start, F, 1, H, C2, 1, 1, GLOWTTS_PERM_NONE, 0, GLOWTTS_BF16, img + 36 * (int64_t)L * S, stride, 0, 0, stream);
    return rc;
}

extern "C" int glowtts_wavenet_bwd(const glowtts_flow_dims* d, const glowtts_flow_params* p, const glowtts_flow_acts* a, const glowtts_flow_grads* g,
                                   void* stream)
{
    if (!d || !p || !a || !g || !p->wn_img_t || !a->rowmask || !g->dx || !g->douts_bf || !g->dskip) return GLOWTTS_E_ARG;
    const int C2 = d->C / 2;
    if (d->precision != GLOWTTS_BF16 || !d->act_bf16 || d->H != WN_H || d->ksize != WN_TAPS || d->L < 1 || d->L > WN_MAXL ||
        (d->C & 7) || C2 <= 64 || C2 > 96 || p->end.npad != 192 || p->in[0].npad != 2 * WN_H) return GLOWTTS_E_ARG;
    if (!g->defer_wgrad || g->pitch_rows || p->cond_rows) return GLOWTTS_E_ARG;
    const bool cnd = g->dcond && p->cond;
    if (cnd && (int64_t)d->B * p->ldcond * 4 >= ((int64_t)1 << 31)) return GLOWTTS_E_ARG;
    const int Tp = d->T + 2 * GLOWTTS_ROW_PAD;
    const int64_t R = (int64_t)d->B * Tp;
    if (R * 2 * WN_H * 2 >= ((int64_t)1 << 31) || R * d->C * 4 >= ((int64_t)1 << 31)) return GLOWTTS_E_ARG;
    wn_bwd_args k;
    memset(&k, 0, sizeof(k));
    k.rows = (int)R; k.rows_per_utt = Tp; k.L = d->L; k.C2 = C2;
    k.wimg = static_cast<const unsigned char*>(p->wn_img_t);
    k.douts_bf = g->douts_bf; k.ldo = p->end.npad; k.rowmask = a->rowmask;
    k.drop_p = d->drop_p; k.seed = d->seed; k.seed_ptr = d->seed_ptr;
    k.dskip = g->dskip; k.ldin = p->in[0].npad; k.dx = g->dx; k.lddx = d->C;
    for (int l = 0; l < d->L; ++l) {
        if (!a->gates[l] || !g->dins[l] || !g->dh[l]) return GLOWTTS_E_ARG;
        k.gates[l] = a->gates[l]; k.dins[l] = g->dins[l]; k.dh[l] = g->dh[l];
        k.dh0_bf16 = g->dh0_bf16;
    }
    const int nvalid = WN_WIN - 2 * WN_PAD * (d->L - 1);
    const dim3 grid((unsigned)((R + nvalid - 1) / nvalid));
    hipStream_t s = static_cast<hipStream_t>(stream);
    if (cnd) { k.dcond = reinterpret_cast<float*>(g->dcond); k.ldcond = p->ldcond; }
#ifdef GLOWTTS_TOOLS
    k.stagger = GLOWTTS_TUNABLE("GLOWTTS_WN_STAGGER", 0);
    if (!cnd && (GLOWTTS_TUNABLE("GLOWTTS_WN_BWD_ABL", 0) & 64)) k.tl = reinterpret_cast<long long*>(g->dcond);
#endif
    if (d->drop_p > 0.f) return cnd ? launch_wn_bwd<true, true>(k, grid, s) : launch_wn_bwd<true, false>(k, grid, s);
    return cnd ? launch_wn_bwd<false, true>(k, grid, s) : launch_wn_bwd<false, false>(k, grid, s);
}
```

glow_tts_amd/decoder.py:

```python
import ctypes
import math

import torch

from . import _lib, abi, ops
from ._lib import c_int, c_void_p
from .abi import FlowActs, FlowDims, FlowGrads, FlowParams, Packed, PrepJob, SumSeg, WgradJob, WnBwdJob

MAXL, ROW_PAD, WN_SLAB = abi.MAX_WN_LAYERS, abi.ROW_PAD, abi.WN_SLAB_BYTES
c_i64 = ctypes.c_int64
_L = _lib.lib


class PrepJobs:
    CAP = abi.PREP_MAX_JOBS

    def __init__(self):
        self.jobs = (PrepJob * self.CAP)()
        self.n, self.blocks, self.max_cols = c_int(0), c_int(0), 1
        self.keep = []

    def add(self, v, g, inv, batch, inner, O, I, taps, transpose, perm, perm_h, packed_ptr, outer_stride, inner_stride=0, w_stride=0, g_stride=0):
        if self.n.value >= self.CAP:
            raise _lib.GlowTTSHipError("too many weight-preparation jobs")
        nb = c_int(0)
        _lib.check(_L().glowtts_prep_job_init(ctypes.byref(self.jobs[self.n.value]), v, g, inv, batch, inner, O, I, taps, int(transpose), perm, perm_h,
                                              packed_ptr, outer_stride, inner_stride, w_stride, g_stride, self.blocks.value, ctypes.byref(nb)), "prep_job_init")
        self.n.value += 1
        self.blocks.value += nb.value
        self.max_cols = max(self.max_cols, I * taps)

    def launch(self, device):
        if self.n.value == 0:
            return
        if TUNE["prep_twin"] and not getattr(self, "_twinned", False):
            _lib.check(_L().glowtts_prep_jobs_twin_in(ctypes.cast(self.jobs, c_void_p), ctypes.byref(self.n), ctypes.byref(self.blocks)), "glowtts_prep_jobs_twin_in")
            self._twinned = True
        _lib.check(_L().glowtts_prep_launch(ctypes.cast(self.jobs, c_void_p), self.n.value, self.blocks.value, self.max_cols, _lib.stream()), "glowtts_prep_launch")


_WSTREAM = {}


def _engine_callbacks_ok():
    return hasattr(torch.autograd.Variable._execution_engine, "queue_callback")


TAIL = {"defer": False, "pending": []}
TUNE = {"chain_actnorm": True, "enc_ln_qkv": True, "enc_proj_ln": True, "wgrad_dma": True, "prep_fused": True, "prep_early": True, "wgrad_wide": True, "fuse_coupling_bwd": True, "act_bf16": True, "fused_wn": True, "fused_wn_bwd": -1, "fused_wn_fwd_skip": -1, "cond_hip": True, "drop_skip32": True, "wgrad_tail_splits": 2, "prep_bwd_late": False, "prep_bwd_gentle": True, "tail_aside": True, "wgrad_balance": False, "prep_twin": True}
STAMPS = {"buf": None, "names": []}


_SEED_STATE = {}


def step_seed(device):
    key = str(device)
    st = _SEED_STATE.get(key)
    capturing = torch.cuda.is_current_stream_capturing()
    if st is None:
        if capturing:
            raise _lib.GlowTTSHipError("run one eager training step before capturing a hipGraph (the dropout seed state is created eagerly)")
        st = _SEED_STATE[key] = torch.zeros(2, dtype=torch.int32, device=device)
        st[1] = int((torch.initial_seed() * 0x9E3779B97F4A7C15 >> 33) & 0x7FFFFFFF)
    if not capturing:
        return torch.randint(0, 2 ** 31 - 1, (1,), device=device, dtype=torch.int32)
    out = torch.empty(1, dtype=torch.int32, device=device)
    _lib.check(_L().glowtts_step_seed(st.data_ptr(), out.data_ptr(), _lib.stream()), "glowtts_step_seed")
    return out


def stamp(name):
    if STAMPS["buf"] is None:
        return
    i = len(STAMPS["names"])
    if i >= STAMPS["buf"].numel():
        return
    STAMPS["names"].append(name)
    _lib.check(_L().glowtts_debug_stamp(STAMPS["buf"].data_ptr() + 8 * i, _lib.stream()), "glowtts_debug_stamp")

TAIL_STACKS = ("start_g", "start_v", "start_b", "rs_g", "rs_v", "rs_b", "rsl_g", "rsl_v", "rsl_b", "end_w", "end_b")


class defer_tail_wgrads:
    def __enter__(self):
        TAIL["defer"], TAIL["pending"] = True, []
        return self

    def __exit__(self, *exc):
        TAIL["defer"] = False
        return False


def flush_tail_wgrads():
    for fn in TAIL["pending"]:
        fn()


def _wgrad_stream(device):
    key = str(device)
    if key not in _WSTREAM:
        _WSTREAM[key] = torch.cuda.Stream(device=device)
    return _WSTREAM[key]


class WgradGroup:

    def __init__(self, rows, taps, precision, xpro=ops.APRO_NONE, io_flags=0, tag="dec", dma_k1=None):
        self.rows, self.taps, self.precision, self.xpro, self.io_flags, self.tag = rows, taps, precision, xpro, io_flags, tag
        self.jobs, self.segments, self._tiles, self._start = [], [], 0, 0
        self.table = None
        self._wide = io_flags in (0, ops.WIO_DY_BF16 | ops.WIO_X_BF16) and xpro == ops.APRO_NONE and precision == ops.BF16 and TUNE["wgrad_wide"]
        self._dma = self._wide and io_flags == (ops.WIO_DY_BF16 | ops.WIO_X_BF16) and bool(TUNE["wgrad_dma"]) and (taps > 1 or bool(dma_k1))

    def add(self, dy, lddy, m, x, ldx, ca, dw, dbias, perm=ops.PERM_NONE, perm_h=0):
        j = WgradJob()
        j.dy, j.x, j.dw, j.dbias, j.lddy, j.ldx = dy, x, dw, dbias, lddy, ldx
        j.m, j.ca, j.xpro, j.perm, j.perm_h = m, ca, self.xpro, perm, perm_h
        if (m | ca | lddy | ldx) & 7 or (dy | x) & 15:
            self._wide = False
        if not self._wide or (self.rows + 512) * max(lddy, ldx) * 2 >= 2 ** 31:
            self._dma = False
        self.jobs.append(j)

    def end_segment(self):
        self.segments.append((self._start, len(self.jobs) - self._start, 0))
        self._start = len(self.jobs)

    def _tile(self):
        dma = self._dma and self._wide
        bm, bn = (192, 192 if self.taps == 1 else 64) if dma else (128, 64)
        for i, (start, n, _) in enumerate(self.segments):
            tiles = 0
            for j in self.jobs[start:start + n]:
                j.mt, j.nt, j.tile0 = (j.m + bm - 1) // bm, (j.ca + bn - 1) // bn, tiles
                tiles += j.mt * j.nt
            self.segments[i] = (start, n, tiles)

    def upload(self, device):
        if not self.jobs:
            return
        self._tile()
        self.table = _lib.staged_upload(bytes((WgradJob * len(self.jobs))(*self.jobs)), device)

    @staticmethod
    def upload_all(groups, device):
        groups = [g for g in groups if g.jobs]
        if not groups:
            return
        for g in groups:
            g._tile()
        raws = [bytes((WgradJob * len(g.jobs))(*g.jobs)) for g in groups]
        table = _lib.staged_upload(b"".join(raws), device)
        off = 0
        for g, r in zip(groups, raws):
            g.table = table[off:off + len(r)]
            off += len(r)

    def balance(self, B, rows_per_utt, device):
        if not (self._dma and self._wide) or len(self.segments) != 0 or self._start != 0 or not self.jobs or self.rows != B * rows_per_utt:
            return False
        cus = torch.cuda.get_device_properties(device).multi_processor_count
        bm, bn = 192, (192 if self.taps == 1 else 64)
        tiles = [((j.m + bm - 1) // bm) * ((j.ca + bn - 1) // bn) for j in self.jobs]
        if len(set(tiles)) != 1 or any(j.dbias is None for j in self.jobs):
            return False
        tpj, nj = tiles[0], len(self.jobs)
        unsplit = float(-(-nj * tpj // cus))
        best = None
        for S in (2, 4, 8, 16):
            if B % S:
                continue
            for a in range(nj, -1, -1):
                W = a * tpj
                if W > cus:
                    continue
                P = (nj - a) * S * tpj
                t, done = (1.0, min(P, (cus - W) * S)) if W else (0.0, 0)
                t += -(-(P - done) // cus) / S
                if best is None or t < best[0] - 1e-9:
                    best = (t, a, S)
        if best is None or best[0] > unsplit - 0.25 or best[1] == nj:
            return False
        _, a, S = best
        whole, cut = self.jobs[:a], self.jobs[a:]
        segs, tot = [], 0
        place = {}
        for j in cut:
            for ptr, n in ((j.dw, j.m * j.ca * self.taps), (j.dbias, j.m)):
                if n % 4 or ptr % 16:
                    return False
                place[ptr] = tot
                if segs and segs[-1][0] + 4 * segs[-1][1] == ptr:
                    segs[-1] = (segs[-1][0], segs[-1][1] + n, segs[-1][2])
                else:
                    segs.append((ptr, n, tot))
                tot += n
        if len(segs) > abi.SUM_MAX_SEGS:
            return False
        self.part = torch.empty(S, tot, device=device)
        Rs = (B // S) * rows_per_utt
        jobs = list(whole)
# ... 589 lines not shown
        else:
            prep = _Prepared(cfg, W, need_bwd=need_bwd, cond=condc, fused_bwd_ok=pitches is None,
                             rows=mels.shape[0] * (mels.shape[2] // cfg.ns + 2 * ROW_PAD), GV=GV)
        ctx.GV = GV
        seed = None
        if drop_p > 0:
            seed, AUX["seed"] = AUX.get("seed"), None
            if seed is None:
                seed = step_seed(mels.device)
        pitch = (pitches.detach(), pitch_w.detach().contiguous(), pitch_b.detach().contiguous()) if pitches is not None else None
        if pitch is not None and condc is None:
            raise _lib.GlowTTSHipError("per-frame pitch conditioning comes with the GR mode's speaker / prosody conditioning (Modules.py:84-90)")
        z, logdet, buf, rowmask, T, prow = _run_forward(cfg, prep, mels.detach(), lengths, drop_p, seed, pitch)
        ctx.drop = (drop_p, seed)
        ctx.prow = prow
        if need_bwd:
            ctx.cfg, ctx.prep, ctx.buf, ctx.rowmask, ctx.T = cfg, prep, buf, rowmask, T
            ctx.lengths, ctx.mel_shape = lengths, mels.shape
            ctx.want_dmel = mels.requires_grad
        z_rows = buf.x[cfg.F]
        ctx.mark_non_differentiable(z_rows)
        ctx.set_materialize_grads(False)
        return z, logdet, z_rows

    @staticmethod
    def backward(ctx, dz, dlogdet, _dz_rows=None):
        L = _L()
        cfg, prep, buf, rowmask, T = ctx.cfg, ctx.prep, ctx.buf, ctx.rowmask, ctx.T
        W = prep.keep
        B, Cm, Tm = ctx.mel_shape
        if dz is None:
            dz = torch.zeros(ctx.mel_shape, device=dlogdet.device)
        dev = dz.device
        prep.launch_bwd_images()
        F_, Lw, H, C = cfg.F, cfg.L, cfg.H, cfg.C
        dx, _, _ = squeeze_rows(cfg, dz.contiguous(), ctx.lengths, want_mask=False)
        R = dx.shape[0]
        dld = dlogdet.contiguous() if dlogdet is not None else torch.zeros(B, device=dev)
        GV = ctx.GV
        from .distributed import register_arena

        def arenas(shapes):
            out = {}
            for tail in (False, True):
                ks = [k for k in shapes if (_TAIL_OF.get(k, False)) == tail]
                sizes = [int(math.prod(shapes[k])) for k in ks]
                padded = [(n + 3) & ~3 for n in sizes]
                flat = (torch.empty if padded == sizes else torch.zeros)(sum(padded), device=dev)
                off = 0
                for k, n, npad in zip(ks, sizes, padded):
                    out[k] = flat[off:off + n].view(shapes[k])
                    off += npad
                if ks:
                    register_arena(*[out[k] for k in ks])
            return out
        ret_shapes = {}
        for k in (WEIGHT_KEYS_GV if GV is not None else WEIGHT_KEYS):
            wk = "w" + k[1:]
            if GV is not None and k[0] in "gv" and wk in GV:
                ret_shapes[k] = tuple(GV[wk][0 if k[0] == "g" else 1].shape)
            else:
                ret_shapes[k] = tuple(W[k].shape)
        RET = arenas(ret_shapes)
        G = {k: (RET[k] if k in RET else torch.empty_like(GV[k][1] if (GV is not None and k in GV) else W[k])) for k in WEIGHT_KEYS}
        d_an = torch.empty(F_, 2 * C + 16, device=dev)
        h0bf = bool(cfg.act_bf16 and buf.xa_bf is not None and buf.skipb is not None)
        douts = None if h0bf else torch.empty(F_, R, prep.ldo, device=dev)
        douts_bf = torch.empty(F_, R, prep.ldo, device=dev, dtype=torch.bfloat16) if cfg.act_bf16 else None
        fuse = TUNE["fuse_coupling_bwd"]
        dins = (torch.empty if prep.ldin == 2 * H else torch.zeros)(F_, Lw, R, prep.ldin, device=dev, dtype=cfg.act_dtype)
        dskip = torch.empty(F_, R, H, device=dev, dtype=cfg.act_dtype)
        dh0 = torch.empty(F_, R, H, device=dev, dtype=cfg.act_dtype if h0bf else torch.float32)
        dhn = torch.empty(F_, max(Lw - 1, 1), R, H, device=dev, dtype=cfg.act_dtype)
        dh_ptr = lambda f, l: dh0[f].data_ptr() if l == 0 else dhn[f, l - 1].data_ptr()
        nscr = L.glowtts_actnorm_stats_scratch_floats(R, C)
        scratch = torch.empty(F_, nscr, device=dev)
        npit = ctx.prow.shape[1] if ctx.prow is not None else 0
        dcond = torch.zeros((B + npit,) + tuple(prep.cond.shape[1:]), device=dev, dtype=torch.int64) if prep.cond is not None else None
        bf = cfg.act_bf16
        gk = WgradGroup(R, cfg.k, cfg.precision, io_flags=(ops.WIO_DY_BF16 | ops.WIO_X_BF16) if bf else 0)
        g1 = WgradGroup(R, 1, cfg.precision)
        S_t = int(TUNE["wgrad_tail_splits"])
        tail_seg = tail_part = tail_fns = None
        if S_t > 1 and h0bf and B % S_t == 0:
            names = ["w_end", "b_end", "w_rs_last", "b_rs_last", "w_start", "b_start"] + (["w_rs", "b_rs"] if Lw > 1 else [])
            if all(G[k].is_contiguous() and G[k].numel() % 4 == 0 and G[k].data_ptr() % 16 == 0 for k in names):
                tot, tail_seg = 0, []
                for k in names:
                    tail_seg.append((G[k].data_ptr(), G[k].numel(), tot))
                    tot += G[k].numel()
                tail_part = torch.empty(S_t, tot, device=dev)
        R_t = R // S_t if tail_seg is not None else R
        gp = WgradGroup(R_t, 1, cfg.precision, ops.APRO_NONE if bf else ops.APRO_PAIRMUL, io_flags=(ops.WIO_DY_BF16 | ops.WIO_X_BF16) if bf else 0,
                        dma_k1=True if tail_seg is not None else None)
        if tail_seg is not None:
            _gp_add = gp.add

            def _split_add(dy, lddy, m, x, ldx, ca, dw, dbias, **kw):
                def image(ptr, s_):
                    for p0, n, off in tail_seg:
                        if p0 <= ptr < p0 + 4 * n:
                            return tail_part.data_ptr() + 4 * (s_ * tail_part.shape[1] + off) + (ptr - p0)
                    raise AssertionError("one-tap weight gradient outside the split's segments")
                for s_ in range(S_t):
                    _gp_add(dy + 2 * s_ * R_t * lddy, lddy, m, x + 2 * s_ * R_t * ldx, ldx, ca, image(dw, s_), image(dbias, s_), **kw)
            gp.add = _split_add
        C2 = C // 2
        order = list(range(F_ - 1, -1, -1))
        for f in order:
            if h0bf:
                gp.add(douts_bf[f].data_ptr(), prep.ldo, prep.ldo, buf.skipb[f].data_ptr(), H, H, G["w_end"][f].data_ptr(), G["b_end"][f].data_ptr(),
                       perm=ops.PERM_PAIR, perm_h=C2)
            else:
                g1.add(douts[f].data_ptr(), prep.ldo, prep.ldo, buf.skip[f].data_ptr(), H, H, G["w_end"][f].data_ptr(), G["b_end"][f].data_ptr(),
                       perm=ops.PERM_PAIR, perm_h=C2)
            for l in range(Lw):
                gates, ldg = (buf.actp[f, l].data_ptr(), H) if bf else (buf.gates[f, l].data_ptr(), 2 * H)
                if l == Lw - 1:
                    gp.add(dskip[f].data_ptr(), H, H, gates, ldg, H, G["w_rs_last"][f].data_ptr(), G["b_rs_last"][f].data_ptr())
                else:
                    gp.add(dh_ptr(f, l + 1), H, H, gates, ldg, H, G["w_rs"][f, l].data_ptr(), G["b_rs"][f, l].data_ptr())
                    gp.add(dskip[f].data_ptr(), H, H, gates, ldg, H, G["w_rs"][f, l].data_ptr() + 4 * H * H, G["b_rs"][f, l].data_ptr() + 4 * H)
                gk.add(dins[f, l].data_ptr(), prep.ldin, prep.ldin, buf.hs[f, l].data_ptr(), H, H, G["w_in"][f, l].data_ptr(), G["b_in"][f, l].data_ptr(),
                       perm=ops.PERM_PAIR, perm_h=H)
            if h0bf:
                gp.add(dh0[f].data_ptr(), H, H, buf.xa_bf[f].data_ptr(), C2, C2, G["w_start"][f].data_ptr(), G["b_start"][f].data_ptr())
            else:
                g1.add(dh0[f].data_ptr(), H, H, buf.xmid[f].data_ptr(), C, C2, G["w_start"][f].data_ptr(), G["b_start"][f].data_ptr())
        if TUNE["wgrad_balance"] and bf:
            gk.balance(B, T + 2 * ROW_PAD, dev)
        for grp in (gk, g1, gp):
            grp.end_segment()
        WgradGroup.upload_all((gk, g1, gp), dev)

        def sum_tail():
            if tail_seg is not None:
                segs = (SumSeg * len(tail_seg))(*[SumSeg(p0, off, n) for p0, n, off in tail_seg])
                _lib.check(L.glowtts_sum_slices_seg(tail_part.data_ptr(), S_t, tail_part.shape[1], segs, len(tail_seg), _lib.stream()), "glowtts_sum_slices_seg")
        main = torch.cuda.current_stream()
        side = _wgrad_stream(dev)
        stamp("dec_bwd_begin")
        nblk_all = L.glowtts_actnorm_bwd_blocks(B * (T + 2 * ROW_PAD))
        assert nblk_all * (2 * C + 16) <= nscr
        for f in order:
            g = FlowGrads()
            g.dx, g.dlogdet, g.douts, g.dskip = dx.data_ptr(), dld.data_ptr(), (douts[f].data_ptr() if douts is not None else None), dskip[f].data_ptr()
            g.douts_bf = douts_bf[f].data_ptr() if douts_bf is not None else None
            g.dh0_bf16 = int(h0bf)
            g.coupling_done = int(fuse and f != order[0])
            if fuse and f > 0:
                g.prev_xmid, g.prev_outs, g.prev_douts = buf.xmid[f - 1].data_ptr(), buf.outs[f - 1].data_ptr(), (douts[f - 1].data_ptr() if douts is not None else None)
                g.prev_douts_bf = douts_bf[f - 1].data_ptr() if douts_bf is not None else None
            g.scratch, g.d_an, g.defer_wgrad = scratch[f].data_ptr(), None, 1
            for l in range(Lw):
                g.dh[l] = dh_ptr(f, l)
                g.dins[l] = dins[f, l].data_ptr()
            if dcond is not None:
                g.dcond = dcond.data_ptr() + 8 * f * Lw * 2 * H
                if npit:
                    g.pitch_rows, g.pitch_ns = ctx.prow.data_ptr(), npit
            acts = buf.acts(f, Lw, rowmask)
            dims = _dims(cfg, B, T, ctx.drop[0], ctx.drop[1], f)
            _lib.check(L.glowtts_flow_backward(ctypes.byref(dims), ctypes.byref(prep.params[f]), ctypes.byref(acts), ctypes.byref(g),
                                               _lib.stream()), "glowtts_flow_backward")
            stamp(f"dec_bwd_flow{f}")
        if TAIL["defer"]:
            gk.launch_segment(0)
            keep = (buf, dins, dskip, dh0, dhn, douts, G)
            TAIL["pending"].append(lambda keep=keep: (gp.launch_segment(0), g1.launch_segment(0), sum_tail()))
        else:
            if dcond is not None and GV is not None and TUNE["tail_aside"] and _engine_callbacks_ok() and _leaf_grads_unset():
                tail_fns = []
            (tail_fns.append if tail_fns is not None else (lambda f: f()))(lambda: [grp.launch_segment(0) for grp in (gk, gp, g1)])
            (tail_fns.append if tail_fns is not None else (lambda f: f()))(sum_tail)
        GVgrad = {}
        if GV is not None:
            wn_now, wn_pending, wn_keep = [], [], []
            for k in WN_KEYS:
                g_, v_ = GV[k]
                if v_.numel() == 0:
                    GVgrad[k] = (torch.zeros_like(g_), torch.zeros_like(v_))
                    continue
                cols = v_.shape[-1] * v_.shape[-2]
                rows_ = v_.numel() // cols
                dv, dg = RET["v" + k[1:]], RET["g" + k[1:]]
                GVgrad[k] = (dg, dv)
                j = WnBwdJob()
                j.dw, j.v, j.g, j.inv_norm, j.dv, j.dg = G[k].data_ptr(), v_.data_ptr(), g_.data_ptr(), prep.inv[k].data_ptr(), dv.data_ptr(), dg.data_ptr()
                j.rows, j.cols = rows_, cols
                wn_keep.append((g_, v_, dv, dg, prep.inv[k], G[k]))
                (wn_pending if (TAIL["defer"] and k != "w_in") else wn_now).append(j)

            def wn_run(jobs, keep=wn_keep):
                if jobs:
                    _lib.check(L.glowtts_weightnorm_bwd_multi((WnBwdJob * len(jobs))(*jobs), len(jobs), _lib.stream()), "glowtts_weightnorm_bwd_multi")
            if wn_pending:
                TAIL["pending"].append(lambda jobs=wn_pending: wn_run(jobs))
            if tail_fns is not None:
                tail_fns.append(lambda jobs=wn_now: wn_run(jobs))
            else:
                wn_run(wn_now)

        def param_sums():
            stamp("dec_wgrads_done")
            _lib.check(L.glowtts_colsum_batched(scratch.data_ptr(), d_an.data_ptr(), nblk_all, 2 * C + 16, F_, nscr, 2 * C + 16, _lib.stream()),
                       "glowtts_colsum_batched")
            _lib.check(L.glowtts_decoder_param_grads(d_an.data_ptr(), dld.data_ptr(), rowmask.data_ptr(), prep.winfo.data_ptr(), G["an_logs"].data_ptr(),
                                                     G["an_bias"].data_ptr(), G["inv_w"].data_ptr(), F_, B, T + 2 * ROW_PAD, C, _lib.stream()),
                       "glowtts_decoder_param_grads")
        if tail_fns is None:
            param_sums()
        else:
            tail_fns.append(param_sums)
            keep = [(buf, dins, dskip, dh0, dhn, douts, douts_bf, G, RET, GV, scratch, d_an, dld, tail_part, gk, gp, g1, prep, rowmask), tail_fns]

            def release():
                if keep[1] is None:
                    return
                fns, keep[1] = keep[1], None
                side.wait_stream(torch.cuda.current_stream(dev))
                with torch.cuda.stream(side):
                    for fn in fns:
                        fn()

            def at_end():
                release()
                main.wait_stream(side)
                keep[0] = None
            release()
            torch.autograd.Variable._execution_engine.queue_callback(at_end)
        dmel = unsqueeze_rows(cfg, dx, ctx.lengths, B, Tm) if ctx.want_dmel else None
        if dcond is not None:
            acc, dcond = dcond.contiguous(), torch.empty(dcond.shape, device=dcond.device)
            _lib.check(_L().glowtts_fx_to_float(acc.data_ptr(), dcond.data_ptr(), acc.numel(), _lib.stream()), "glowtts_fx_to_float")
        dpw = dpb = None
        if ctx.prow is not None:
            dpb = dcond[:B].sum(0).view(F_, Lw, 2 * H)
            dpw = dcond[B:].view(npit, F_, Lw, 2 * H).permute(1, 2, 3, 0).contiguous()
            dcond = dcond[:B]
        if GV is not None:
            out = []
            for k in WEIGHT_KEYS_GV:
                wk = "w" + k[1:]
                if k[0] in "gv" and wk in GVgrad:
                    out.append(GVgrad[wk][0 if k[0] == "g" else 1])
                else:
                    out.append(G[k].view_as(W[k]))
            return (None, dmel, None, dcond, None, None, dpw, dpb) + tuple(out)
        return (None, dmel, None, dcond, None, None, dpw, dpb) + tuple(G[k].view_as(W[k]) for k in WEIGHT_KEYS)


def _wn(g, v):
    return g * v / v.flatten(-2).norm(dim=-1).unsqueeze(-1).unsqueeze(-1)


def stack_decoder_weights(P, cfg, prefix="layer_Dict.Decoder.layer_Dict.Flows"):
    F_, L = cfg.F, cfg.L
    fl = lambda f: f"{prefix}.{f}.layers"
    wn = lambda f, name: (P[f"{fl(f)}.2.layer_Dict.{name}.weight_g"], P[f"{fl(f)}.2.layer_Dict.{name}.weight_v"],
                          P[f"{fl(f)}.2.layer_Dict.{name}.bias"])
    an_logs = torch.stack([P[f"{fl(f)}.0.logs"].reshape(-1) for f in range(F_)])
    an_bias = torch.stack([P[f"{fl(f)}.0.bias"].reshape(-1) for f in range(F_)])
    inv_w = torch.stack([P[f"{fl(f)}.1.weight"] for f in range(F_)])
    st = [wn(f, "Start") for f in range(F_)]
    w_start = _wn(torch.stack([t[0] for t in st]), torch.stack([t[1] for t in st]))
    b_start = torch.stack([t[2] for t in st])
    ins = [[wn(f, f"WaveNet.layer_Dict.In_{l}") for l in range(L)] for f in range(F_)]
    w_in = _wn(torch.stack([torch.stack([t[0] for t in row]) for row in ins]), torch.stack([torch.stack([t[1] for t in row]) for row in ins]))
    b_in = torch.stack([torch.stack([t[2] for t in row]) for row in ins])
    rs = [[wn(f, f"WaveNet.layer_Dict.Res_Skip_{l}") for l in range(L)] for f in range(F_)]
    if L > 1:
        w_rs = _wn(torch.stack([torch.stack([t[0] for t in row[:-1]]) for row in rs]), torch.stack([torch.stack([t[1] for t in row[:-1]]) for row in rs]))
        b_rs = torch.stack([torch.stack([t[2] for t in row[:-1]]) for row in rs])
    else:
        dev = w_in.device
        w_rs, b_rs = torch.zeros(F_, 0, 2 * cfg.H, cfg.H, 1, device=dev), torch.zeros(F_, 0, 2 * cfg.H, device=dev)
    w_rs_last = _wn(torch.stack([row[-1][0] for row in rs]), torch.stack([row[-1][1] for row in rs]))
    b_rs_last = torch.stack([row[-1][2] for row in rs])
    w_end = torch.stack([P[f"{fl(f)}.2.layer_Dict.End.weight"] for f in range(F_)])
    b_end = torch.stack([P[f"{fl(f)}.2.layer_Dict.End.bias"] for f in range(F_)])
    return (an_logs, an_bias, inv_w, w_start, b_start, w_in, b_in, w_rs, b_rs, w_rs_last, b_rs_last, w_end, b_end)


class _StackedLeaves(torch.autograd.Function):
    @staticmethod
    def forward(ctx, flat, *leaves):
        ctx.n, ctx.leaf_shape = len(leaves), leaves[0].shape
        return flat.detach()

    @staticmethod
    def backward(ctx, g):
        g = g.contiguous().view(ctx.n, *ctx.leaf_shape)
        return (None,) + tuple(g.unbind(0))


class LeafStack:

    def __init__(self, leaves, lead):
        self.leaves, self.lead = list(leaves), tuple(lead)
        assert len(self.leaves) == int(torch.tensor(self.lead).prod()) and len({tuple(t.shape) for t in self.leaves}) == 1
        self.flat = None

    def _aliased(self):
        f = self.flat
        if f is None or f.device != self.leaves[0].device:
            return False
# ... 191 lines not shown
```

include/glowtts_hip.h:

```cpp
#ifndef GLOWTTS_HIP_H
#define GLOWTTS_HIP_H
#include <stdint.h>

#ifdef __cplusplus
extern "C" {
#endif

#define GLOWTTS_OK            0
#define GLOWTTS_E_ARG        -1
#define GLOWTTS_E_LAUNCH     -2
#define GLOWTTS_ABI_VERSION    7

int glowtts_abi_version(void);
int glowtts_device_arch(char *buf, int buflen);

int64_t glowtts_launch_count(const char *kernel_class);
void glowtts_launch_log_reset(void);
int glowtts_launch_log_dump(char *buf, int buflen);

int glowtts_mfma_clock_probe(long long *out, int nwg, int iters, int *wall_khz, void *stream);
int glowtts_debug_stamp(long long *slot, void *stream);
int glowtts_step_seed(uint32_t *state, uint32_t *out, void *stream);

int glowtts_mas_dp_f32(const float *value, const int32_t *t_xs, const int32_t *t_ys,
// ... 98 lines not shown
    float *out0; int64_t ld0;
    float *out1; int64_t ld1;
    const float *in0; int64_t ldi0;
    int batch;
    int64_t a_bstride, w_bstride , bias_bstride, out_bstride, mask_bstride;
    const int32_t *ncols_valid;
    uint32_t seed; float drop_p;
    const uint32_t *seed_ptr;
    int io_flags;
} glowtts_conv_args;

int glowtts_conv_chain(const glowtts_conv_args *first, const glowtts_conv_args *second, void *stream);
int glowtts_conv_cl(const glowtts_conv_args *args , void *stream);

#define GLOWTTS_ROW_PAD 2

int glowtts_squeeze_rows(const float *mel, float *rows, float *rowmask, const int64_t *lengths,
                         int B, int Cm, int Tm, int ns, void *stream);
int glowtts_unsqueeze_rows(const float *rows, float *mel, const int64_t *lengths,
                           int B, int Cm, int Tm, int ns, int use_fill, float fill, void *stream);
int glowtts_inv1x1_prepare(const float *W, float *winfo, int F, void *stream);
int glowtts_actnorm_inv1x1(const float *xin, float *xout, const float *logs, const float *bias,
                           const float *winfo, const float *rowmask, int64_t rows, int C, int reverse, void *stream);
int glowtts_actnorm_inv1x1_pass_bf(const float *xin, float *xout, float *xpass, void *xa_bf, const float *logs, const float *bias, const float *winfo,
                                   const float *rowmask, int64_t rows, int C, void *stream);
int glowtts_actnorm_inv1x1_pass(const float *xin, float *xout, float *xpass, const float *logs, const float *bias, const float *winfo,
                                const float *rowmask, int64_t rows, int C, void *stream);
int glowtts_actnorm_stats(const float *x, const float *rowmask, float *stats, float *scratch,
                          int64_t rows, int C, void *stream);
int64_t glowtts_actnorm_stats_scratch_floats(int64_t rows, int C);
int glowtts_actnorm_from_stats(const float *stats, float *logs, float *bias, int C, void *stream);
int glowtts_coupling_bwd(float *dz, const float *xmid, const float *outs, float *douts, const float *rowmask,
                         const float *dlogdet, int64_t rows, int C, int ldo, int rows_per_utt, void *stream);
int glowtts_coupling_bwd_bf16(float *dz, const float *xmid, const float *outs, float *douts, void *douts_bf16, const float *rowmask,
                              const float *dlogdet, int64_t rows, int C, int ldo, int rows_per_utt, void *stream);
int glowtts_fill_zero(float *p, int64_t n, void *stream);
int glowtts_actnorm_inv1x1_bwd(const float *dz, float *dx, const float *x, const float *logs, const float *bias,
                               const float *winfo, const float *rowmask, float *param_grads, float *scratch,
                               int64_t rows, int C, void *stream);
int64_t glowtts_actnorm_bwd_blocks(int64_t rows);
int glowtts_actnorm_inv1x1_bwd_coupling(const float *dz, float *dx, const float *x, const float *logs, const float *bias, const float *winfo,
                                        const float *rowmask, float *scratch, int64_t rows, int C,
                                        const float *prev_xmid, const float *prev_outs, float *prev_douts, void *prev_douts_bf16,
                                        const float *dlogdet, int ldo, int rows_per_utt, void *stream);
int glowtts_colsum_batched(const float *partial, float *out, int nrows, int n, int batch, int64_t part_stride, int64_t out_stride, void *stream);
int glowtts_decoder_param_grads(const float *d_an, const float *dlogdet, const float *rowmask, const float *winfo,
                                float *dlogs, float *dbias, float *dw, int F, int B, int Tp, int C, void *stream);
int glowtts_decoder_logdet(const float *outs_all, int64_t flow_stride, const float *logs_all, const float *winfo_all,
                           const float *rowmask, float *part, float *logdet, int F, int B, int Tp, int C, int ldo, void *stream);

typedef struct glowtts_wgrad_args {
    const float *dy; int64_t lddy;
    const float *x;  int64_t ldx;
    int xpro;
    const float *xmask;
    int rows, m, ca, taps, pad;
    int perm, perm_h;
    int precision;
    int splits, accumulate;
    float *dw;
    float *dbias;
    int io_flags;
} glowtts_wgrad_args;
#define GLOWTTS_WIO_DY_BF16 1
#define GLOWTTS_WIO_X_BF16  2
#define GLOWTTS_WIO_WIDE    4
#define GLOWTTS_WIO_DMA     8
int glowtts_wgrad_cl(const glowtts_wgrad_args *args , void *stream);

typedef struct glowtts_wgrad_job {
    const float *dy; const float *x; const float *xmask; float *dw; float *dbias;
    int64_t lddy, ldx;
    int m, ca, xpro, perm, perm_h;
    int tile0, mt, nt;
    int rows;
    int reserved;
} glowtts_wgrad_job;
int glowtts_wgrad_grouped(const glowtts_wgrad_job *dev_jobs, int njobs, int total_tiles, int rows, int taps, int pad,
                          int xpro, int precision, int splits, int accumulate, void *stream);
int glowtts_wgrad_grouped_io(const glowtts_wgrad_job *dev_jobs, int njobs, int total_tiles, int rows, int taps, int pad,
                             int xpro, int precision, int splits, int accumulate, int io_flags, void *stream);

int glowtts_wgrad_grouped_phased(const glowtts_wgrad_job *dev_jobs, int njobs, int total_tiles, int whole_tiles, int rows, int taps, void *stream);

#define GLOWTTS_MAX_WN_LAYERS 8

typedef struct glowtts_packed {
    const void *w; int npad, kchunks;
} glowtts_packed;

typedef struct glowtts_flow_dims {
    int B, T;
    int C;
    int H;
    int L;
    int ksize;
    int precision;
    float drop_p;
    uint32_t seed;
    const uint32_t *seed_ptr;
    int act_bf16;
} glowtts_flow_dims;

typedef struct glowtts_flow_params {
    const float *an_logs, *an_bias;
    const float *winfo;
    glowtts_packed start, in[GLOWTTS_MAX_WN_LAYERS], rs[GLOWTTS_MAX_WN_LAYERS], end;
    glowtts_packed start_t, in_t[GLOWTTS_MAX_WN_LAYERS], rs_t[GLOWTTS_MAX_WN_LAYERS], end_t;
    const float *b_start, *b_in[GLOWTTS_MAX_WN_LAYERS], *b_rs[GLOWTTS_MAX_WN_LAYERS], *b_end;
    const float *cond; int64_t ldcond;
    int cond_rows;
    const void *wn_img, *wn_img_t;
} glowtts_flow_params;

typedef struct glowtts_flow_acts {
    float *xin;
    float *xmid;
    float *xout;
    float *hs[GLOWTTS_MAX_WN_LAYERS];
    float *gates[GLOWTTS_MAX_WN_LAYERS];
    float *skip;
    float *outs;
    const float *rowmask;
    float *acts[GLOWTTS_MAX_WN_LAYERS];
    float *skip_bf;
    void *xa_bf;
    const float *next_an_logs, *next_an_bias, *next_winfo;
    float *next_xmid, *next_xout;
    void *next_xa_bf;
    int actnorm_done;
} glowtts_flow_acts;

typedef struct glowtts_flow_grads {
    float *dx;
    const float *dlogdet;
    float *douts;
    float *dskip;
    float *dh[GLOWTTS_MAX_WN_LAYERS];
    float *dins[GLOWTTS_MAX_WN_LAYERS];
    int defer_wgrad;
    float *scratch;
    float *d_an;
    float *dw_start, *db_start;
    float *dw_in[GLOWTTS_MAX_WN_LAYERS], *db_in[GLOWTTS_MAX_WN_LAYERS];
    float *dw_rs[GLOWTTS_MAX_WN_LAYERS], *db_rs[GLOWTTS_MAX_WN_LAYERS];
    float *dw_end, *db_end;
    int64_t *dcond;
    float *douts_bf;
    int coupling_done;
    const float *prev_xmid, *prev_outs;
    float *prev_douts, *prev_douts_bf;
    const float *pitch_rows; int pitch_ns;
    int dh0_bf16;
} glowtts_flow_grads;

int glowtts_flow_forward(const glowtts_flow_dims *d, const glowtts_flow_params *p, const glowtts_flow_acts *a, void *stream);
int glowtts_flow_inverse(const glowtts_flow_dims *d, const glowtts_flow_params *p, const glowtts_flow_acts *a, void *stream);
int glowtts_flow_encode(const glowtts_flow_dims *d, const glowtts_flow_params *p, const glowtts_flow_acts *a, void *stream);
int glowtts_flow_backward(const glowtts_flow_dims *d, const glowtts_flow_params *p, const glowtts_flow_acts *a,
                          const glowtts_flow_grads *g, void *stream);
#define GLOWTTS_WN_SLAB_BYTES 24576
#define GLOWTTS_WN_FUSED_MAX_LAYERS 4
int glowtts_wavenet_image_bytes(int L, int transposed, int64_t *bytes_out );
int glowtts_wavenet_pack_images(const float *w_start, const float *w_in, const float *w_rs, const float *w_rs_last, const float *w_end,
                                int F, int L, int C2, void *img_fwd, void *img_bwd, void *stream);
int glowtts_wavenet_prep_jobs(glowtts_prep_job *jobs, int max_jobs, int *njobs, int *block,
                              const float *v_start, const float *g_start, float *inv_start, const float *v_in, const float *g_in, float *inv_in,
                              const float *v_rs, const float *g_rs, float *inv_rs, const float *v_rsl, const float *g_rsl, float *inv_rsl,
                              const float *w_end, int F, int L, int C2, void *img_fwd, int F_bwd, void *img_bwd);
int glowtts_wavenet_fwd(const glowtts_flow_dims *d, const glowtts_flow_params *p, const glowtts_flow_acts *a,
                        const float *xsrc, float *xdst, int reverse, int keep, void *stream);
int glowtts_wavenet_bwd(const glowtts_flow_dims *d, const glowtts_flow_params *p, const glowtts_flow_acts *a, const glowtts_flow_grads *g,
                        void *stream);

void glowtts_wavenet_debug_safe_waits(int on);

int glowtts_utt_colsum(const float *x, int64_t ldx, float *out, int64_t ldout, int B, int rows_per_utt, int n,
                       int perm, int perm_h, void *stream);

int glowtts_cond_linear_fwd(const float *v, const float *g, const float *bias, const float *vec, float *out, float *inv_out,
                            int N, int D, int B, int accumulate, void *stream);
int64_t glowtts_cond_linear_bwd_scratch_floats(int N, int D, int B);
int glowtts_cond_linear_supported(int N, int D, int B);
int glowtts_fx_to_float(const int64_t *acc, float *out, int64_t n, void *stream);
int glowtts_cond_linear_bwd(const float *dcond, int64_t ldd, const float *v, const float *g, const float *inv, const float *vec,
                            float *dv, float *dg, float *dbias, float *dvec, float *scratch, int N, int D, int B, void *stream);

int glowtts_gru_fwd(const float *gi, const float *w_hh, const float *b_hh, float *hs, float *keep, int B, int T, int H, void *stream);
int glowtts_gru_bwd(const float *dhs, const float *hs, const float *keep, const float *w_hh, float *dgi, float *dgh,
                    int B, int T, int H, void *stream);
int glowtts_gst_supported(int B, int Tp, int G, int C, int H, int NT, int I);
int64_t glowtts_gst_keep_floats(int B, int G, int C, int H, int NT, int I);
int glowtts_gst_fwd(const float *hs, const int64_t *lengths, int stride_prod, const float *tokens, const float *Wq, const float *bq, const float *Wk,
                    const float *bk, const float *Wv, const float *bv, const float *Wp, const float *bp, float *K, float *V, float *out, float *keep,
                    int B, int Tp, int G, int C, int H, int NT, int I, void *stream);
int glowtts_gst_bwd(const float *dout, const float *keep, const int64_t *lengths, int stride_prod, const float *tokens, const float *Wq, const float *Wk,
                    const float *Wv, const float *Wp, const float *K, const float *V, float *dhs, float *scratch,
                    float *dWq, float *dbq, float *dWk, float *dbk, float *dWv, float *dbv, float *dWp, float *dbp, float *dtokens,
                    int B, int Tp, int G, int C, int H, int NT, int I, void *stream);

typedef struct glowtts_c2d_pack_job {
    const float *w; void *img;
    int Ci, Co, cls, N, K, npad, kchunks, block0;
} glowtts_c2d_pack_job;
int glowtts_conv3x3s2_supported(int B, int H, int W, int Ci, int Co);
int glowtts_conv3x3s2_image_bytes(int Ci, int Co, int precision, int64_t *fwd_bytes , int64_t *dgrad_bytes );
int glowtts_conv3x3s2_pack_job_init(glowtts_c2d_pack_job *job , const float *w, int Ci, int Co, int cls, int precision, void *img,
                                    int block0, int *blocks_out );
int glowtts_conv3x3s2_pack(const glowtts_c2d_pack_job *dev_jobs, int njobs, int total_blocks, int precision, void *stream);
int glowtts_conv3x3s2_fwd(const float *x, const float *w, const void *img_fwd, float *y, int B, int H, int W, int Ci, int Co, int relu,
                          int precision, void *stream);
int glowtts_conv3x3s2_dgrad(const float *dpre, const void *const *img_dgrad, const float *gate, float *dx, int B, int H, int W, int Ci, int Co,
                            int precision, void *stream);
#define GLOWTTS_C2D_MAX_LAYERS 8
typedef struct glowtts_c2d_reduce_job { const float *partial; float *dw; int splits, Ci, Co, block0 ; } glowtts_c2d_reduce_job;
int64_t glowtts_conv3x3s2_wgrad_scratch_floats(int B, int H, int W, int Ci, int Co);
int glowtts_conv3x3s2_wgrad(const float *x, const float *dpre, float *partial, int B, int H, int W, int Ci, int Co, int precision,
                            int *splits_out , void *stream);
int glowtts_conv3x3s2_wgrad_reduce(const glowtts_c2d_reduce_job *jobs , int njobs, void *stream);

int glowtts_layernorm_fwd(const float *a, const float *b, float *s_out, const float *gamma, const float *beta, const float *rowmask,
                          float *y, float *stats, int64_t rows, int C, float eps, int relu, float drop_p, uint32_t seed,
                          const uint32_t *seed_ptr, void *stream);
int glowtts_layernorm_fwd_io(const float *a, const float *b, float *s_out, const float *gamma, const float *beta, const float *rowmask,
                             float *y, float *stats, int64_t rows, int C, float eps, int relu, float drop_p, uint32_t seed,
                             const uint32_t *seed_ptr, uint16_t *y_bf16, void *stream);
int glowtts_proj_layernorm(const float *a, int64_t lda, const void *w, int npad, const float *bias, const float *x, const float *gamma,
                           const float *beta, const float *rowmask, float *proj_kept, float *s, float *stats, float *y, uint16_t *y_bf16,
                           int64_t rows, int C, float eps, float drop_p, uint32_t seed, const uint32_t *seed_ptr, void *stream);
int glowtts_layernorm_qkv(const float *a, const float *b, const float *gamma, const float *beta, const float *rowmask, float *s, float *stats,
                          float *y, uint16_t *y_bf16, const void *wqkv, int npad, const float *bias, float *qkv, int64_t rows, int C, float eps,
                          void *stream);
int64_t glowtts_layernorm_scratch_floats(int64_t rows, int C);
int glowtts_layernorm_bwd(const float *dy, const float *y, const float *s, const float *stats, const float *gamma, const float *rowmask,
                          float *ds, float *dgamma_dbeta, float *scratch, int64_t rows, int C, int gated, float drop_p, void *stream);
int glowtts_layernorm_bwd_io(const float *dy, const float *y, const float *s, const float *stats, const float *gamma, const float *rowmask,
                             float *ds, float *dgamma_dbeta, float *scratch, int64_t rows, int C, int gated, float drop_p,
                             uint16_t *ds_bf16, const float *gate_out, float gate_scale, void *stream);
int glowtts_gate_bwd(const float *dy, const float *out, const float *rowmask, float *dz, int64_t rows, int C, float scale, void *stream);
int glowtts_gate_bwd_io(const void *dy, const void *out, const float *rowmask, void *dz, int64_t rows, int C, float scale, int io_flags, void *stream);
int glowtts_token_masks(const int64_t *lengths, float *mask, float *rowmask, int B, int T, void *stream);
int glowtts_embedding_fwd(const int64_t *tokens, const float *table, const float *rowmask, float *rows, int B, int T, int C, float scale, void *stream);
int glowtts_embedding_bwd(const int64_t *tokens, const float *drows, const float *rowmask, float *dtable, int V, int B, int T, int C, float scale, void *stream);
int glowtts_rpr_attention_fwd(const float *qkv, const float *relk, const float *relv, const float *rowmask, float *out, float *P,
                              int B, int Tp, int H, int D, int win, float drop_p, uint32_t seed, const uint32_t *seed_ptr, void *stream);
int64_t glowtts_rpr_attention_scratch_floats(int B, int Tp, int H, int D, int win);
int glowtts_rpr_attention_bwd(const float *qkv, const float *relk, const float *relv, const float *rowmask, const float *P, const float *dout,
                              float *dS, float *dqkv, float *drelk, float *drelv, float *scratch,
                              int B, int Tp, int H, int D, int win, float drop_p, uint32_t seed, const uint32_t *seed_ptr, void *stream);
int glowtts_rpr_attention_fwd_prec(const float *qkv, const float *relk, const float *relv, const float *rowmask, float *out, float *P,
                                   int B, int Tp, int H, int D, int win, float drop_p, uint32_t seed, const uint32_t *seed_ptr, int precision, void *stream);
int64_t glowtts_rpr_attention_bwd_partial_rows(int B, int Tp, int H, int D, int win);
int glowtts_rpr_attention_fwd_eval(const float *qkv, const float *relk, const float *relv, const float *rowmask, float *out,
                                   int B, int Tp, int H, int D, int win, int precision, void *stream);
int glowtts_rpr_attention_bwd_prec(const float *qkv, const float *relk, const float *relv, const float *rowmask, const float *P, const float *dout,
                                   float *dS, float *dqkv, float *drelk, float *drelv, float *scratch,
                                   int B, int Tp, int H, int D, int win, float drop_p, uint32_t seed, const uint32_t *seed_ptr, int precision, void *stream);

int glowtts_logprior_prep(const float *mean, const float *log_std, const int64_t *token_lengths, const int64_t *mel_lengths, float *packed,
                          float *cb, float *fmask, int32_t *tx32, int32_t *ty32, int B, int Cm, int Tx, int Ty, int mel_multiple,
                          int *npad_out, int *kchunks_out, void *stream);
int glowtts_expand_fwd(const float *src, const int32_t *idx, float *out, int B, int C, int Tx, int Ty, void *stream);
int glowtts_expand_bwd(const float *dout, const int32_t *idx, float *dsrc, int B, int C, int Tx, int Ty, void *stream);
int glowtts_duration_targets(const int32_t *idx, const int64_t *token_lengths, float *out, int B, int Tx, int Ty, void *stream);
int glowtts_mle_loss_fwd(const float *z, const float *mean, const float *log_std, const float *log_dets, const int64_t *lengths,
                         float *loss, float *inv_denom, float *scratch, int64_t n, int B, int n_squeeze, int mel_dim, void *stream);
int glowtts_mle_loss_bwd(const float *z, const float *mean, const float *log_std, const float *dloss, const float *inv_denom,
                         float *dz, float *dmean, float *dlog_std, int64_t n, float *dlogdet, int B, void *stream);
int glowtts_expand_pair_targets(const float *mean, const float *log_std, const int32_t *idx, const int64_t *token_lengths, float *mel_mean,
                                float *mel_log_std, float *targets, float *path, int B, int C, int Tx, int Ty, void *stream);
int glowtts_prior_loss_bwd(const float *z, const float *mean, const float *log_std, const int32_t *idx, const float *dloss, const float *inv_denom,
                           float *dz, float *dmean, float *dlog_std, float *dlogdet, int B, int C, int Tx, int Ty, void *stream);
int glowtts_mse_loss_fwd(const float *a, const float *target, float *loss, int64_t n, float scale, const int64_t *lengths, int B, const float *extent,
                         float *da_unit, void *stream);
int glowtts_mse_loss_bwd(const float *a, const float *target, const float *dloss, float *da, int64_t n, float scale, const int64_t *lengths, int B,
                         const float *extent, void *stream);
int glowtts_prior_loss(const float *z, const float *mel_mean, const float *mel_log_std, const float *mean, const float *log_std, const int32_t *idx,
                       const float *log_dets, const int64_t *lengths, const float *dloss, float *scratch, uint32_t *counter, float *loss, float *inv_denom,
                       float *dz, float *dmean, float *dlog_std, float *dlogdet, int B, int C, int Tx, int Ty, int n_squeeze, int mel_dim, void *stream);
int glowtts_dur_proj_supported(int C);
int glowtts_dur_proj_fwd(const float *d, const float *w, const float *bias, const float *mask, float *out, int B, int T, int pad, int C, void *stream);
int glowtts_dur_proj_bwd(const float *g, const float *mask, const float *d, const float *w, float *dd, float *dw, float *dbias, float *scratch,
                         uint32_t *counter, int B, int T, int pad, int C, void *stream);
int glowtts_prior_split_fwd(const float *rows, float *mean, float *log_std, int B, int T, int pad, int M, void *stream);
int glowtts_prior_split_bwd(const float *dmean, const float *dlog_std, float *drows, int B, int T, int pad, int M, void *stream);

int glowtts_weightnorm_fwd(const float *v, const float *g, float *w, float *inv_norm, int64_t rows, int cols, void *stream);
int glowtts_weightnorm_bwd(const float *dw, const float *v, const float *g, const float *inv_norm, float *dv, float *dg,
                           int64_t rows, int cols, void *stream);
#define GLOWTTS_WN_BWD_MAX_JOBS 8
typedef struct glowtts_wn_bwd_job {
    const float *dw, *v, *g, *inv_norm; float *dv, *dg;
    int64_t rows; int cols, reserved;
} glowtts_wn_bwd_job;
int glowtts_weightnorm_bwd_multi(const glowtts_wn_bwd_job *jobs, int njobs, void *stream);

typedef struct glowtts_opt_job {
    float *p; const float *g; float *m; float *v;
    int64_t n;
    int64_t block0;
} glowtts_opt_job;
int glowtts_opt_chunk(void);
int glowtts_multi_grad_norm(const glowtts_opt_job *dev_jobs, int njobs, int total_blocks, float max_norm, float *partial,
                            float *norm_and_coef, void *stream);
int glowtts_sum_slices(const float *partial, float *out, int S, int64_t n, void *stream);
#define GLOWTTS_SUM_MAX_SEGS 12
typedef struct glowtts_sum_seg { float *dst; int64_t off, n; } glowtts_sum_seg;
int glowtts_sum_slices_seg(const float *partial, int S, int64_t stride, const glowtts_sum_seg *segs , int nseg, void *stream);
int glowtts_multi_grad_scale(const glowtts_opt_job *dev_jobs, int njobs, int total_blocks, const float *coef, void *stream);
int glowtts_radam_step(const glowtts_opt_job *dev_jobs, int njobs, int total_blocks, const float *hyper, const float *grad_scale, void *stream);

int glowtts_vocoder_supported(int n_fft, int win_length, int hop);
int glowtts_mel_to_linear_f32(const float *mels, const int32_t *frame_lengths, const float *basis, float *mag, int B, int Mel, int T, int F, float max_abs,
                              void *stream);
int glowtts_stft_f32(const float *wav, const int32_t *wav_lengths, const float *window, const float *twiddle, float *spec, int B, int ldx, int T, int n_fft,
                     int win_length, int hop, void *stream);
int glowtts_istft_f32(const float *spec, const int32_t *frame_lengths, const float *window, const float *twiddle, float *frames, float *wav, int B, int T,
                      int ldx, int n_fft, int win_length, int hop, void *stream);
int glowtts_overlap_add_f32(const float *frames, const int32_t *frame_lengths, const float *window, float *wav, int B, int T, int ldx, int n_fft,
                            int win_length, int hop, void *stream);
int glowtts_griffin_lim_step_f32(const float *x, const float *x_prev, const float *mag, const int32_t *frame_lengths, const float *window,
                                 const float *twiddle, float alpha, float *frames, int B, int T, int ldx, int n_fft, int win_length, int hop, void *stream);

int glowtts_mel_analysis_f32(const float *wav, const int32_t *wav_lengths, const float *window, const float *twiddle, const int32_t *fb_index,
                             const float *fb_weight, float *mel, int B, int ldx, int T, int Mel, int n_weights, int n_fft, int win_length, int hop,
                             float pre_emphasis, float min_db, float max_abs, void *stream);
// ... 48 lines not shown
```

Baseline: 5.498 million mel-frames/s.

## Fold actnorm/inv1x1 backward and prior coupling backward into fused WaveNet bwd kernel

Moves the actnorm + invertible 1x1 backward (and the previous flow's coupling backward) into the epilogue of the fused WaveNet backward kernel, so dx for the first half-channels is taken straight from LDS and per-block parameter-gradient partials are written to scratch. The goal is to drop a separate kernel launch and a full re-read and re-write of dx per flow step. The shared per-row math is factored into a host/device helper and checked by a new host test. The cost is extra registers and LDS reduction work in an already heavy kernel, which may lower occupancy. Padding rows of the partial buffer are zeroed so the block count matches the downstream reduction.

```diff
diff --git a/glow_tts_amd/abi.py b/glow_tts_amd/abi.py
--- a/glow_tts_amd/abi.py
+++ b/glow_tts_amd/abi.py
@@ -61,7 +61,7 @@
     _fields_ = _fields(("dx dlogdet douts dskip", P), ("dh dins", P * MAX_WN_LAYERS), ("defer_wgrad", I),
                        ("scratch d_an dw_start db_start", P), ("dw_in db_in dw_rs db_rs", P * MAX_WN_LAYERS),
                        ("dw_end db_end dcond douts_bf", P), ("coupling_done", I), ("prev_xmid prev_outs prev_douts prev_douts_bf pitch_rows", P),
-                       ("pitch_ns dh0_bf16", I))
+                       ("pitch_ns dh0_bf16 fold_actnorm an_rows", I))
 
 
 class WnBwdJob(ctypes.Structure):
@@ -177,6 +177,8 @@
     "glowtts_wavenet_prep_jobs": (I, [P, I, PI, PI] + [P] * 13 + [I] * 3 + [P, I, P]),
     "glowtts_wavenet_fwd": (I, [P] * 5 + [I, I, P]),
     "glowtts_wavenet_bwd": (I, [P] * 5),
+    "glowtts_wavenet_bwd_folds": (I, [P] * 4),
+    "glowtts_wavenet_bwd_blocks": (L, [L, I]),
     "glowtts_wavenet_debug_safe_waits": (None, [I]),
     "glowtts_utt_colsum": (I, [P, L, P, L] + [I] * 5 + [P]),
     "glowtts_cond_linear_fwd": (I, [P] * 6 + [I] * 4 + [P]),
diff --git a/glow_tts_amd/csrc/actnorm_math.h b/glow_tts_amd/csrc/actnorm_math.h
--- a/glow_tts_amd/csrc/actnorm_math.h
+++ b/glow_tts_amd/csrc/actnorm_math.h
@@ -1,4 +1,12 @@
 #pragma once
+#include <math.h>
+#if defined(__HIPCC__)
+#define AN_HD __host__ __device__ __forceinline__
+#else
+#define AN_HD inline
+#endif
+
+#if defined(__HIPCC__)
 __device__ __forceinline__ void actnorm_mix4(const float (&x)[4], const float (&e)[4], const float (&b)[4], const float (&w)[16], float m, float (&o)[4])
 {
     float v[4];
@@ -8,3 +16,34 @@
     for (int k = 0; k < 4; ++k)
         o[k] = __builtin_fmaf(w[k * 4 + 3], v[3], __builtin_fmaf(w[k * 4 + 2], v[2], __builtin_fmaf(w[k * 4 + 1], v[1], w[k * 4 + 0] * v[0]))) * m;
 }
+#endif
+
+AN_HD void actnorm_bwd_row8(const float (&w)[16], const float (&el)[8], const float (&bs)[8], float m, const float (&dz)[8], const float (&xv)[8],
+                            bool coupled, const float (&lg)[4], const float (&xb)[4], float dl,
+                            float (&o)[8], float (&dm)[4], float (&dg)[4], float (&accW)[16], float (&accL)[8], float (&accB)[8])
+{
+    const float dv[8] = {dz[0] * m, dz[1] * m, dz[2] * m, dz[3] * m, dz[4] * m, dz[5] * m, dz[6] * m, dz[7] * m};
+#pragma unroll
+    for (int e = 0; e < 2; ++e) {
+        const int sl[4] = {2 * e, 2 * e + 1, 4 + 2 * e, 5 + 2 * e};
+        float y[4], dy[4];
+#pragma unroll
+        for (int k = 0; k < 4; ++k) y[k] = (bs[sl[k]] + el[sl[k]] * xv[sl[k]]) * m;
+#pragma unroll
+        for (int k = 0; k < 4; ++k)
+            dy[k] = (w[0 * 4 + k] * dv[sl[0]] + w[1 * 4 + k] * dv[sl[1]] + w[2 * 4 + k] * dv[sl[2]] + w[3 * 4 + k] * dv[sl[3]]) * m;
+#pragma unroll
+        for (int a = 0; a < 4; ++a)
+#pragma unroll
+            for (int k = 0; k < 4; ++k) accW[a * 4 + k] += dv[sl[a]] * y[k];
+#pragma unroll
+        for (int k = 0; k < 4; ++k) { o[sl[k]] = dy[k] * el[sl[k]]; accL[sl[k]] += o[sl[k]] * xv[sl[k]]; accB[sl[k]] += dy[k]; }
+    }
+    if (coupled) {
+#pragma unroll
+        for (int k = 0; k < 4; ++k) {
+            const float d = o[4 + k], e = expf(lg[k]);
+            dm[k] = d * m; dg[k] = (d * e * xb[k] + dl) * m; o[4 + k] = d * e * m;
+        }
+    }
+}
diff --git a/glow_tts_amd/csrc/flow.hip b/glow_tts_amd/csrc/flow.hip
--- a/glow_tts_amd/csrc/flow.hip
+++ b/glow_tts_amd/csrc/flow.hip
@@ -211,8 +211,11 @@
     else if (dbf) CHECK(glowtts_coupling_bwd_bf16(g->dx, a->xmid, a->outs, g->douts, g->douts_bf, a->rowmask, g->dlogdet, R, C, ldo, c.Tp, stream));
     else     CHECK(glowtts_coupling_bwd(g->dx, a->xmid, a->outs, g->douts, a->rowmask, g->dlogdet, R, C, ldo, c.Tp, stream));
     if (p->wn_img_t) {
-        CHECK(glowtts_wavenet_bwd(d, p, a, g, stream));
         if (g->prev_outs && g->d_an) return GLOWTTS_E_ARG;
+        if (glowtts_wavenet_bwd_folds(d, p, a, g)) return glowtts_wavenet_bwd(d, p, a, g, stream);
+        glowtts_flow_grads gu = *g;
+        gu.fold_actnorm = 0;
+        CHECK(glowtts_wavenet_bwd(d, p, a, &gu, stream));
         if (g->prev_outs)
             return glowtts_actnorm_inv1x1_bwd_coupling(g->dx, g->dx, a->xin, p->an_logs, p->an_bias, p->winfo, a->rowmask, g->scratch, R, C,
                                                        g->prev_xmid, g->prev_outs, g->prev_douts, g->prev_douts_bf, g->dlogdet, ldo, c.Tp, stream);
diff --git a/glow_tts_amd/csrc/flow_ops.hip b/glow_tts_amd/csrc/flow_ops.hip
--- a/glow_tts_amd/csrc/flow_ops.hip
+++ b/glow_tts_amd/csrc/flow_ops.hip
@@ -357,34 +357,13 @@
                 xb = *reinterpret_cast<const float4*>(nc.xmid + r * C + C2 + 4 * q);
                 dl = nc.dld[r / nc.rows_per_utt];
             }
-            const float dv[8] = {dlo.x * m, dlo.y * m, dlo.z * m, dlo.w * m, dhi.x * m, dhi.y * m, dhi.z * m, dhi.w * m};
+            const float dzv[8] = {dlo.x, dlo.y, dlo.z, dlo.w, dhi.x, dhi.y, dhi.z, dhi.w};
             const float xv[8] = {xlo.x, xlo.y, xlo.z, xlo.w, xhi.x, xhi.y, xhi.z, xhi.w};
-            float o[8];
-#pragma unroll
-            for (int e = 0; e < 2; ++e) {
-                const int sl[4] = {2 * e, 2 * e + 1, 4 + 2 * e, 5 + 2 * e};
-                float y[4], dy[4];
-#pragma unroll
-                for (int k = 0; k < 4; ++k) y[k] = (bs[sl[k]] + el[sl[k]] * xv[sl[k]]) * m;
-#pragma unroll
-                for (int k = 0; k < 4; ++k)
-                    dy[k] = (w[0 * 4 + k] * dv[sl[0]] + w[1 * 4 + k] * dv[sl[1]] + w[2 * 4 + k] * dv[sl[2]] + w[3 * 4 + k] * dv[sl[3]]) * m;
-#pragma unroll
-                for (int a = 0; a < 4; ++a)
-#pragma unroll
-                    for (int k = 0; k < 4; ++k) accW[a * 4 + k] += dv[sl[a]] * y[k];
-#pragma unroll
-                for (int k = 0; k < 4; ++k) { o[sl[k]] = dy[k] * el[sl[k]]; accL[sl[k]] += o[sl[k]] * xv[sl[k]]; accB[sl[k]] += dy[k]; }
-            }
+            const float lgv[4] = {lg.x, lg.y, lg.z, lg.w}, xbv[4] = {xb.x, xb.y, xb.z, xb.w};
+            float o[8], dm[4], dg[4];
+            actnorm_bwd_row8(w, el, bs, m, dzv, xv, nc.outs != nullptr, lgv, xbv, dl, o, dm, dg, accW, accL, accB);
             *reinterpret_cast<float4*>(dx + r * C + 4 * q) = make_float4(o[0], o[1], o[2], o[3]);
             if (nc.outs) {
-                const float lgv[4] = {lg.x, lg.y, lg.z, lg.w}, xbv[4] = {xb.x, xb.y, xb.z, xb.w};
-                float dm[4], dg[4], ob[4];
-#pragma unroll
-                for (int k = 0; k < 4; ++k) {
-                    const float d = o[4 + k], e = expf(lgv[k]);
-                    dm[k] = d * m; dg[k] = (d * e * xbv[k] + dl) * m; ob[k] = d * e * m;
-                }
                 float* dob = nc.douts ? nc.douts + r * nc.ldo : nullptr;
                 if (dob) {
                     *reinterpret_cast<float4*>(dob + pc) = make_float4(dm[0], dm[1], dm[2], dm[3]);
@@ -409,10 +388,8 @@
                         *reinterpret_cast<uint2*>(nc.douts16 + r * nc.ldo + pp + 32) = make_uint2(0u, 0u);
                     }
                 }
-                *reinterpret_cast<float4*>(dx + r * C + C2 + 4 * q) = make_float4(ob[0], ob[1], ob[2], ob[3]);
-            } else {
-                *reinterpret_cast<float4*>(dx + r * C + C2 + 4 * q) = make_float4(o[4], o[5], o[6], o[7]);
             }
+            *reinterpret_cast<float4*>(dx + r * C + C2 + 4 * q) = make_float4(o[4], o[5], o[6], o[7]);
         }
     }
     float* out = partial + (long)blockIdx.x * (2 * C + 16);
diff --git a/glow_tts_amd/csrc/host_tests/actnorm_fold_host.cpp b/glow_tts_amd/csrc/host_tests/actnorm_fold_host.cpp
--- /dev/null
+++ b/glow_tts_amd/csrc/host_tests/actnorm_fold_host.cpp
@@ -0,0 +1,200 @@
+#include <math.h>
+#include <stdint.h>
+#include <stdio.h>
+#include <vector>
+#include "../actnorm_math.h"
+
+namespace {
+
+constexpr int WIN = 64, PAD = 2, NT = 768, XS = 100;
+constexpr double EPS32 = 5.9604644775390625e-08;
+
+struct Rng {
+    uint64_t s;
+    double uni() { s = s * 6364136223846793005ull + 1442695040888963407ull; return (double)(s >> 11) / 9007199254740992.0; }
+    float sym(float a) { return (float)((2.0 * uni() - 1.0) * a); }
+};
+
+int pair_col(int j) { return (j >> 5) * 64 + (j & 31); }
+
+struct Case { int B, T, C, L; bool coupled, keep32; int an_rows; };
+
+int run_case(const Case& cs)
+{
+    const int C = cs.C, C2 = C / 2, Q = C / 8, Tp = cs.T + 2 * PAD, rows = cs.B * Tp, ldo = (C + 63) / 64 * 64, n = 2 * C + 16;
+    const int halo = PAD * (cs.L - 1), nvalid = WIN - 2 * halo, grid = (rows + nvalid - 1) / nvalid;
+    const int an_rows = cs.an_rows > grid ? cs.an_rows : grid;
+    Rng g{(uint64_t)(rows * 131 + C)};
+    std::vector<float> mask(rows), dz((size_t)rows * C), xin((size_t)rows * C), xmid((size_t)rows * C), outs((size_t)rows * ldo), dld(cs.B), logs(C), bias(C), w(16);
+    for (int b = 0; b < cs.B; ++b) {
+        const int len = b == cs.B - 1 && cs.B > 2 ? 0 : cs.T - 5 * b;
+        for (int t = 0; t < Tp; ++t) mask[b * Tp + t] = (t >= PAD && t < PAD + len) ? 1.f : 0.f;
+        dld[b] = g.sym(1.f) + 0.25f * b;
+    }
+    for (int r = 0; r < rows; ++r) {
+        const bool bad = mask[r] == 0.f;
+        for (int c = 0; c < C; ++c) {
+            const float junk = ((r + c) & 1) ? -1e3f : 1e3f;
+            dz[(size_t)r * C + c] = bad ? junk : g.sym(1.7f);
+            xin[(size_t)r * C + c] = bad ? junk : g.sym(2.5f);
+            xmid[(size_t)r * C + c] = bad ? junk : g.sym(2.5f);
+        }
+        for (int c = 0; c < ldo; ++c) outs[(size_t)r * ldo + c] = 1e3f;
+        for (int j = 0; j < C2; ++j) { outs[(size_t)r * ldo + pair_col(j)] = g.sym(1.7f); outs[(size_t)r * ldo + pair_col(j) + 32] = bad ? 20.f : g.sym(0.5f); }
+    }
+    for (int c = 0; c < C; ++c) { logs[c] = g.sym(0.5f); bias[c] = g.sym(0.8f); }
+    for (int i = 0; i < 16; ++i) w[i] = (i % 5 == 0 ? 1.f : 0.f) + g.sym(0.3f);
+
+    std::vector<float> dx = dz;
+    std::vector<float> douts((size_t)rows * ldo, 7.f);
+    std::vector<float> douts16((size_t)rows * ldo, 7.f);
+    std::vector<float> partial((size_t)an_rows * n, 1e30f);
+    std::vector<int> written((size_t)rows * C, 0);
+    for (int blk = 0; blk < grid; ++blk) {
+        const int v0 = blk * nvalid, lim = rows - v0 < nvalid ? rows - v0 : nvalid;
+        std::vector<float> XA((size_t)WIN * XS, 1e30f), red((size_t)32 * NT, 1e30f);
+        for (int wrow = 0; wrow < WIN; ++wrow) {
+            const int r = wrow - halo;
+            if (r < 0 || r >= lim) continue;
+            for (int ch = 0; ch < 96; ++ch) if (ch < C2) XA[(size_t)r * XS + ch] = dx[(size_t)(v0 + r) * C + ch];
+        }
+        const int tpq = NT / Q;
+        for (int tid = 0; tid < NT; ++tid) {
+            const int q = tid % Q, rl = tid / Q;
+            float el[8], bs[8], accW[16] = {0}, accL[8] = {0}, accB[8] = {0};
+            for (int k = 0; k < 4; ++k) { el[k] = expf(logs[4 * q + k]); el[4 + k] = expf(logs[C2 + 4 * q + k]); bs[k] = bias[4 * q + k]; bs[4 + k] = bias[C2 + 4 * q + k]; }
+            const float (&wm)[16] = *reinterpret_cast<const float (*)[16]>(w.data());
+            const int j0 = 4 * q, pc = pair_col(j0);
+            if (rl < tpq) {
+                for (int r = rl; r < lim; r += tpq) {
+                    const size_t gr = (size_t)(v0 + r);
+                    float dzv[8], xv[8], lg[4] = {0, 0, 0, 0}, xb[4] = {0, 0, 0, 0}, dl = 0.f, o[8], dm[4], dg[4];
+                    for (int k = 0; k < 4; ++k) {
+                        dzv[k] = XA[(size_t)r * XS + 4 * q + k]; dzv[4 + k] = dx[gr * C + C2 + 4 * q + k];
+                        xv[k] = xin[gr * C + 4 * q + k]; xv[4 + k] = xin[gr * C + C2 + 4 * q + k];
+                        if (cs.coupled) { lg[k] = outs[gr * ldo + pc + 32 + k]; xb[k] = xmid[gr * C + C2 + 4 * q + k]; }
+                    }
+                    if (cs.coupled) dl = dld[gr / Tp];
+                    actnorm_bwd_row8(wm, el, bs, mask[gr], dzv, xv, cs.coupled, lg, xb, dl, o, dm, dg, accW, accL, accB);
+                    for (int k = 0; k < 4; ++k) {
+                        dx[gr * C + 4 * q + k] = o[k]; dx[gr * C + C2 + 4 * q + k] = o[4 + k];
+                        ++written[gr * C + 4 * q + k]; ++written[gr * C + C2 + 4 * q + k];
+                    }
+                    if (cs.coupled) {
+                        for (int k = 0; k < 4; ++k) {
+                            if (cs.keep32) { douts[gr * ldo + pc + k] = dm[k]; douts[gr * ldo + pc + 32 + k] = dg[k]; }
+                            douts16[gr * ldo + pc + k] = dm[k]; douts16[gr * ldo + pc + 32 + k] = dg[k];
+                        }
+                        for (int jp = C2 + j0; jp < ldo / 2; jp += C2) {
+                            const int pp = pair_col(jp);
+                            for (int k = 0; k < 4; ++k) {
+                                if (cs.keep32) { douts[gr * ldo + pp + k] = 0.f; douts[gr * ldo + pp + 32 + k] = 0.f; }
+                                douts16[gr * ldo + pp + k] = 0.f; douts16[gr * ldo + pp + 32 + k] = 0.f;
+                            }
+                        }
+                    }
+                }
+            }
+            for (int i = 0; i < 32; ++i) {
+                const float v = i < 16 ? accW[i] : (i < 24 ? accL[i - 16] : accB[i - 24]);
+                red[(size_t)i * NT + tid] = rl < tpq ? v : 0.f;
+            }
+        }
+        float* out = &partial[(size_t)blk * n];
+        for (int e = 0; e < 16; ++e) {
+            float s[16];
+            for (int part = 0; part < 16; ++part) { s[part] = 0.f; for (int t = 0; t < NT / 16; ++t) s[part] += red[(size_t)e * NT + t * 16 + part]; }
+            for (int o = 8; o >= 1; o >>= 1) { float t2[16]; for (int l = 0; l < 16; ++l) t2[l] = s[l] + s[l ^ o]; for (int l = 0; l < 16; ++l) s[l] = t2[l]; }
+            out[2 * C + e] = s[0];
+        }
+        for (int tid = 0; tid < 16 * Q; ++tid) {
+            const int which = tid / (8 * Q), sl = (tid / Q) % 8, qq = tid % Q;
+            float s = 0.f;
+            for (int t = qq; t < tpq * Q; t += Q) s += red[(size_t)(16 + which * 8 + sl) * NT + t];
+            out[which * C + (sl < 4 ? 4 * qq + sl : C2 + 4 * qq + sl - 4)] = s;
+        }
+        for (int row = grid + blk; row < an_rows; row += grid) for (int i = 0; i < n; ++i) partial[(size_t)row * n + i] = 0.f;
+    }
+    std::vector<float> d_an(n);
+    for (int i = 0; i < n; ++i) {
+        float s[64];
+        for (int lane = 0; lane < 64; ++lane) { s[lane] = 0.f; for (int k = lane; k < an_rows; k += 64) s[lane] += partial[(size_t)k * n + i]; }
+        for (int o = 32; o > 0; o >>= 1) for (int l = 0; l + o < 64; ++l) if (l < o) s[l] += s[l + o];
+        d_an[i] = s[0];
+    }
+
+    int bad = 0;
+    auto fail = [&](const char* what, long i, long j, double got, double want, double bar) {
+        if (bad++ < 5) fprintf(stderr, "  %s[%ld][%ld]: got %.9g want %.9g bar %.3g\n", what, i, j, got, want, bar);
+    };
+    std::vector<double> rW(16, 0.0), aW(16, 0.0), rL(C, 0.0), aL(C, 0.0), rB(C, 0.0), aB(C, 0.0);
+    for (int r = 0; r < rows; ++r) {
+        const double m = mask[r];
+        for (int c = 0; c < C; ++c) if (written[(size_t)r * C + c] != 1) fail("dx written count", r, c, written[(size_t)r * C + c], 1, 0);
+        for (int gq = 0; gq < C / 4; ++gq) {
+            const int ch[4] = {2 * gq, 2 * gq + 1, C2 + 2 * gq, C2 + 2 * gq + 1};
+            double d[4], y[4], ya[4];
+            for (int k = 0; k < 4; ++k) {
+                d[k] = (double)dz[(size_t)r * C + ch[k]] * m;
+                const double ex = exp((double)logs[ch[k]]) * xin[(size_t)r * C + ch[k]];
+                y[k] = ((double)bias[ch[k]] + ex) * m; ya[k] = (fabs((double)bias[ch[k]]) + fabs(ex)) * m;
+            }
+            for (int k = 0; k < 4; ++k) {
+                double dy = 0, dya = 0;
+                for (int a = 0; a < 4; ++a) { dy += (double)w[a * 4 + k] * d[a]; dya += fabs((double)w[a * 4 + k] * d[a]); }
+                dy *= m; dya *= m;
+                const double e = exp((double)logs[ch[k]]), o = dy * e, oa = dya * e;
+                rL[ch[k]] += o * xin[(size_t)r * C + ch[k]]; aL[ch[k]] += oa * fabs((double)xin[(size_t)r * C + ch[k]]);
+                rB[ch[k]] += dy; aB[ch[k]] += dya;
+                for (int a = 0; a < 4; ++a) { rW[a * 4 + k] += d[a] * y[k]; aW[a * 4 + k] += fabs(d[a]) * ya[k]; }
+                double want = o, scale = oa;
+                if (cs.coupled && k >= 2) {
+                    const int j = 2 * gq + (k - 2);
+                    const double ec = exp((double)outs[(size_t)r * ldo + pair_col(j) + 32]), xbv = xmid[(size_t)r * C + C2 + j];
+                    want = o * ec * m; scale = oa * ec * m;
+                    const double wm_ = o * m, wg = (o * ec * xbv + (double)dld[r / Tp]) * m, sg = (oa * ec * fabs(xbv) + fabs((double)dld[r / Tp])) * m;
+                    for (int cp = 0; cp < 2; ++cp) {
+                        const float* dst = cp ? douts16.data() : douts.data();
+                        if (!cp && !cs.keep32) continue;
+                        const double g0 = dst[(size_t)r * ldo + pair_col(j)], g1 = dst[(size_t)r * ldo + pair_col(j) + 32];
+                        if (!(fabs(g0 - wm_) <= 16 * EPS32 * oa * m)) fail("dm", r, j, g0, wm_, 16 * EPS32 * oa * m);
+                        if (!(fabs(g1 - wg) <= 16 * EPS32 * sg)) fail("dlogs_c", r, j, g1, wg, 16 * EPS32 * sg);
+                    }
+                }
+                const double got = dx[(size_t)r * C + ch[k]];
+                if (!(fabs(got - want) <= 16 * EPS32 * scale)) fail("dx", r, ch[k], got, want, 16 * EPS32 * scale);
+            }
+        }
+        if (cs.coupled) {
+            std::vector<char> used(ldo, 0);
+            for (int j = 0; j < C2; ++j) { used[pair_col(j)] = 1; used[pair_col(j) + 32] = 1; }
+            for (int c = 0; c < ldo; ++c) if (!used[c]) {
+                if (douts16[(size_t)r * ldo + c] != 0.f) fail("pad16", r, c, douts16[(size_t)r * ldo + c], 0, 0);
+                if (cs.keep32 && douts[(size_t)r * ldo + c] != 0.f) fail("pad32", r, c, douts[(size_t)r * ldo + c], 0, 0);
+            }
+        }
+    }
+    for (int c = 0; c < C; ++c) {
+        if (!(fabs(d_an[c] - rL[c]) <= 1e-5 * aL[c])) fail("dlogs", 0, c, d_an[c], rL[c], 1e-5 * aL[c]);
+        if (!(fabs(d_an[C + c] - rB[c]) <= 1e-5 * aB[c])) fail("dbias", 0, c, d_an[C + c], rB[c], 1e-5 * aB[c]);
+    }
+    for (int i = 0; i < 16; ++i) if (!(fabs(d_an[2 * C + i] - rW[i]) <= 1e-5 * aW[i])) fail("dW", 0, i, d_an[2 * C + i], rW[i], 1e-5 * aW[i]);
+    printf("case B=%d T=%d C=%d L=%d coupled=%d fp32=%d rows=%d grid=%d an_rows=%d: %s\n", cs.B, cs.T, C, cs.L, (int)cs.coupled, (int)cs.keep32, rows, grid, an_rows,
+           bad ? "FAILED" : "passed");
+    return bad;
+}
+
+}
+
+int main()
+{
+    const Case cases[] = {
+        {3, 37, 160, 4, true, true, 4}, {3, 37, 160, 4, true, false, 0}, {3, 37, 136, 4, true, true, 8}, {3, 37, 136, 1, true, false, 4},
+        {3, 37, 160, 1, false, false, 4}, {3, 37, 136, 4, false, false, 3}, {1, 9, 192, 4, true, true, 1}, {2, 64, 144, 2, true, true, 5},
+    };
+    int bad = 0;
+    for (const Case& c : cases) bad += run_case(c);
+    if (bad) { printf("%d mismatches\n", bad); return 1; }
+    printf("ok\n");
+    return 0;
+}
diff --git a/glow_tts_amd/csrc/wavenet_fused_bwd.hip b/glow_tts_amd/csrc/wavenet_fused_bwd.hip
--- a/glow_tts_amd/csrc/wavenet_fused_bwd.hip
+++ b/glow_tts_amd/csrc/wavenet_fused_bwd.hip
@@ -5,6 +5,7 @@
 #include "tunable.h"
 #include "launch_log.h"
 #include "wavenet_common.h"
+#include "actnorm_math.h"
 
 int glowtts_wavenet_safe_waits_flag();
 
@@ -23,6 +24,9 @@
 constexpr int BW_LDS = BOFF_P3 + WN_KCH * 4 * 64;
 static_assert(BW_LDS <= 160 * 1024, "LDS budget");
 static_assert(BSZ_T >= WN_NW * 8 * 256, "the partial-sum exchange (8 registers per wave and round) reuses the gate-gradient tile");
+constexpr int AN_XS = 100;
+static_assert(WN_WIN * AN_XS * 4 <= BSZ_T, "the d x_a rows fit the d skip tile");
+static_assert(BOFF_DT + 32 * WN_NT * 4 <= BOFF_MK, "the accumulators end in front of the row masks");
 
 struct wn_bwd_args {
     int rows, rows_per_utt, L, C2;
@@ -37,6 +41,8 @@
     int dh0_bf16;
     float* dx; int64_t lddx;
     float* dcond; int64_t ldcond;
+    const float* an_xin; const float* an_logs; const float* an_bias; const float* an_winfo; float* an_partial; int an_rows, C;
+    const float* nc_xmid; const float* nc_outs; float* nc_douts; void* nc_douts16; const float* nc_dld;
     long long* tl;
     int stagger;
 };
@@ -513,6 +519,7 @@
         }
     }
     TLS();
+    const bool fold = p.an_xin != nullptr;
     if (cf < 3) {
         int rb = rbw;
         asm volatile("" : "+v"(rb));
@@ -532,21 +539,140 @@
                     old[h][rt][i] = __uint_as_float(__builtin_amdgcn_raw_buffer_load_b32(rx, ok ? vx0 + (uint32_t)(c * (int)p.lddx * 4) : OOB, 0, 0));
                 }
         }
-#pragma unroll
-        for (int h = 0; h < 2; ++h) {
-            const bool cok = jch0 + 16 * h < p.C2;
-            const uint32_t vx0 = (uint32_t)((t0 + rb) * (int)p.lddx + jch0 + 16 * h) * 4u;
-#pragma unroll
-            for (int rt = 0; rt < 2; ++rt)
-#pragma unroll
-                for (int i = 0; i < 4; ++i) {
-                    const int c = 16 * rt + i;
-                    const bool ok = cok && own0 + (uint32_t)c < (uint32_t)lim;
-                    if constexpr (!(ABL & 4)) __builtin_amdgcn_raw_buffer_store_b32(__float_as_uint(old[h][rt][i] + acc[rt][h][i]), rx, ok ? vx0 + (uint32_t)(c * (int)p.lddx * 4) : OOB, 0, 0);
-                }
+        if (fold) {
+            float* const XA = reinterpret_cast<float*>(DS);
+#pragma unroll
+            for (int h = 0; h < 2; ++h) {
+                const bool cok = jch0 + 16 * h < p.C2;
+#pragma unroll
+                for (int rt = 0; rt < 2; ++rt)
+#pragma unroll
+                    for (int i = 0; i < 4; ++i) {
+                        const uint32_t r = own0 + (uint32_t)(16 * rt + i);
+                        if (cok && r < (uint32_t)lim) XA[r * AN_XS + jch0 + 16 * h] = old[h][rt][i] + acc[rt][h][i];
+                    }
+            }
+        } else {
+#pragma unroll
+            for (int h = 0; h < 2; ++h) {
+                const bool cok = jch0 + 16 * h < p.C2;
+                const uint32_t vx0 = (uint32_t)((t0 + rb) * (int)p.lddx + jch0 + 16 * h) * 4u;
+#pragma unroll
+                for (int rt = 0; rt < 2; ++rt)
+#pragma unroll
+                    for (int i = 0; i < 4; ++i) {
+                        const int c = 16 * rt + i;
+                        const bool ok = cok && own0 + (uint32_t)c < (uint32_t)lim;
+                        if constexpr (!(ABL & 4)) __builtin_amdgcn_raw_buffer_store_b32(__float_as_uint(old[h][rt][i] + acc[rt][h][i]), rx, ok ? vx0 + (uint32_t)(c * (int)p.lddx * 4) : OOB, 0, 0);
+                    }
+            }
         }
     }
     TLS();
+    if (fold) {
+        __syncthreads();
+        const float* const XA = reinterpret_cast<const float*>(DS);
+        float* const red = reinterpret_cast<float*>(DT);
+        int tidp = tid;
+        asm volatile("" : "+v"(tidp));
+        const int C = p.C, C2 = p.C2, Q = C >> 3;
+        const int tpq = WN_NT / Q;
+        const int q = tidp % Q, rl = tidp / Q;
+        float w[16];
+#pragma unroll
+        for (int i = 0; i < 16; ++i) w[i] = p.an_winfo[i];
+        float accW[16], accL[8], accB[8];
+#pragma unroll
+        for (int i = 0; i < 16; ++i) accW[i] = 0.f;
+#pragma unroll
+        for (int i = 0; i < 8; ++i) { accL[i] = 0.f; accB[i] = 0.f; }
+        float el[8], bs[8];
+        {
+            const float4 la = *reinterpret_cast<const float4*>(p.an_logs + 4 * q), lb = *reinterpret_cast<const float4*>(p.an_logs + C2 + 4 * q);
+            const float4 ba = *reinterpret_cast<const float4*>(p.an_bias + 4 * q), bb = *reinterpret_cast<const float4*>(p.an_bias + C2 + 4 * q);
+            const float lv[8] = {la.x, la.y, la.z, la.w, lb.x, lb.y, lb.z, lb.w}, bv[8] = {ba.x, ba.y, ba.z, ba.w, bb.x, bb.y, bb.z, bb.w};
+#pragma unroll
+            for (int k = 0; k < 8; ++k) { el[k] = expf(lv[k]); bs[k] = bv[k]; }
+        }
+        const bool coupled = p.nc_outs != nullptr;
+        const int ldo = (int)p.ldo;
+        const int j0 = 4 * q, pc = (j0 >> 5) * 64 + (j0 & 31);
+        if (rl < tpq) {
+            for (int r = rl; r < lim; r += tpq) {
+                const long g = v0 + r;
+                const float m = MK[halo + WN_PAD + r];
+                const float4 dlo = *reinterpret_cast<const float4*>(XA + r * AN_XS + 4 * q);
+                float* const dxr = p.dx + g * C;
+                const float4 dhi = *reinterpret_cast<const float4*>(dxr + C2 + 4 * q);
+                const float4 xlo = *reinterpret_cast<const float4*>(p.an_xin + g * C + 4 * q), xhi = *reinterpret_cast<const float4*>(p.an_xin + g * C + C2 + 4 * q);
+                float4 lg = make_float4(0.f, 0.f, 0.f, 0.f), xb = lg;
+                float dl = 0.f;
+                if (coupled) {
+                    lg = *reinterpret_cast<const float4*>(p.nc_outs + g * ldo + pc + 32);
+                    xb = *reinterpret_cast<const float4*>(p.nc_xmid + g * C + C2 + 4 * q);
+                    dl = p.nc_dld[g / p.rows_per_utt];
+                }
+                const float dzv[8] = {dlo.x, dlo.y, dlo.z, dlo.w, dhi.x, dhi.y, dhi.z, dhi.w};
+                const float xv[8] = {xlo.x, xlo.y, xlo.z, xlo.w, xhi.x, xhi.y, xhi.z, xhi.w};
+                const float lgv[4] = {lg.x, lg.y, lg.z, lg.w}, xbv[4] = {xb.x, xb.y, xb.z, xb.w};
+                float o[8], dm[4], dg[4];
+                actnorm_bwd_row8(w, el, bs, m, dzv, xv, coupled, lgv, xbv, dl, o, dm, dg, accW, accL, accB);
+                *reinterpret_cast<float4*>(dxr + 4 * q) = make_float4(o[0], o[1], o[2], o[3]);
+                *reinterpret_cast<float4*>(dxr + C2 + 4 * q) = make_float4(o[4], o[5], o[6], o[7]);
+                if (coupled) {
+                    float* const dob = p.nc_douts ? p.nc_douts + g * ldo : nullptr;
+                    __bf16* const dob16 = p.nc_douts16 ? static_cast<__bf16*>(p.nc_douts16) + g * ldo : nullptr;
+                    if (dob) {
+                        *reinterpret_cast<float4*>(dob + pc) = make_float4(dm[0], dm[1], dm[2], dm[3]);
+                        *reinterpret_cast<float4*>(dob + pc + 32) = make_float4(dg[0], dg[1], dg[2], dg[3]);
+                    }
+                    typedef __bf16 bf4 __attribute__((ext_vector_type(4)));
+                    if (dob16) {
+                        bf4 a, b;
+#pragma unroll
+                        for (int k = 0; k < 4; ++k) { a[k] = (__bf16)dm[k]; b[k] = (__bf16)dg[k]; }
+                        *reinterpret_cast<bf4*>(dob16 + pc) = a;
+                        *reinterpret_cast<bf4*>(dob16 + pc + 32) = b;
+                    }
+                    for (int jp = C2 + j0; jp < ldo / 2; jp += C2) {
+                        const int pp = (jp >> 5) * 64 + (jp & 31);
+                        if (dob) {
+                            *reinterpret_cast<float4*>(dob + pp) = make_float4(0.f, 0.f, 0.f, 0.f);
+                            *reinterpret_cast<float4*>(dob + pp + 32) = make_float4(0.f, 0.f, 0.f, 0.f);
+                        }
+                        if (dob16) {
+                            *reinterpret_cast<uint2*>(dob16 + pp) = make_uint2(0u, 0u);
+                            *reinterpret_cast<uint2*>(dob16 + pp + 32) = make_uint2(0u, 0u);
+                        }
+                    }
+                }
+            }
+        }
+#pragma unroll
+        for (int i = 0; i < 32; ++i) {
+            const float v = (i < 16) ? accW[i] : (i < 24 ? accL[i - 16] : accB[i - 24]);
+            red[i * WN_NT + tidp] = (rl < tpq) ? v : 0.f;
+        }
+        __syncthreads();
+        const int n = 2 * C + 16;
+        float* const out = p.an_partial + (long)blockIdx.x * n;
+        if (tidp >= 512) {
+            const int e = (tidp - 512) >> 4, part = tidp & 15;
+            float s = 0.f;
+            for (int t = 0; t < WN_NT / 16; ++t) s += red[e * WN_NT + t * 16 + part];
+#pragma unroll
+            for (int o = 8; o >= 1; o >>= 1) s += __shfl_xor(s, o, 16);
+            if (part == 0) out[2 * C + e] = s;
+        } else if (tidp < 16 * Q) {
+            const int which = tidp / (8 * Q), sl = (tidp / Q) % 8, qq = tidp % Q;
+            float s = 0.f;
+            for (int t = qq; t < tpq * Q; t += Q) s += red[(16 + which * 8 + sl) * WN_NT + t];
+            const int c = (sl < 4) ? (4 * qq + sl) : (C2 + 4 * qq + (sl - 4));
+            out[which * C + c] = s;
+        }
+        for (int row = (int)gridDim.x + (int)blockIdx.x; row < p.an_rows; row += (int)gridDim.x)
+            for (int i = tidp; i < n; i += WN_NT) p.an_partial[(long)row * n + i] = 0.f;
+    }
 }
 
 template <bool DROP, bool COND, int ABL = 0>
@@ -580,6 +706,7 @@
         attr_done = true;
     }
     GLOWTTS_NOTE_STATIC("wn_bwd<%s%s>", DROP ? "drop" : "nodrop", COND ? ",cond" : "");
+    if (k.an_xin) GLOWTTS_NOTE_STATIC("wn_bwd_an<%s%s>", DROP ? "drop" : "nodrop", COND ? ",cond" : "");
     hipLaunchKernelGGL((wn_bwd_kernel<DROP, COND, ABL>), grid, dim3(WN_NT), BW_LDS, s, k);
     return hipGetLastError() == hipSuccess ? GLOWTTS_OK : GLOWTTS_E_LAUNCH;
 }
@@ -601,6 +728,28 @@
                                          img + (42 + 36 * (int64_t)(L - 2) + 15 * half) * S, stride, -36 * S, (int64_t)2 * H * H * WN_TAPS, stream);
     if (rc == GLOWTTS_OK) rc = glowtts_pack_weight_strided(w_start, F, 1, H, C2, 1, 1, GLOWTTS_PERM_NONE, 0, GLOWTTS_BF16, img + 36 * (int64_t)L * S, stride, 0, 0, stream);
     return rc;
+}
+
+extern "C" int64_t glowtts_wavenet_bwd_blocks(int64_t rows, int L)
+{
+    if (rows < 1 || L < 1 || L > WN_MAXL) return 0;
+    const int nvalid = WN_WIN - 2 * WN_PAD * (L - 1);
+    return (rows + nvalid - 1) / nvalid;
+}
+
+extern "C" int glowtts_wavenet_bwd_folds(const glowtts_flow_dims* d, const glowtts_flow_params* p, const glowtts_flow_acts* a, const glowtts_flow_grads* g)
+{
+    if (!d || !p || !a || !g || !g->fold_actnorm || g->d_an || !g->scratch || !g->dx || !a->xin || !a->rowmask || !p->an_logs || !p->an_bias || !p->winfo) return 0;
+    if ((d->C & 7) || d->L < 1 || d->L > WN_MAXL) return 0;
+    const int64_t R = (int64_t)d->B * (d->T + 2 * GLOWTTS_ROW_PAD);
+    if (g->an_rows && g->an_rows < glowtts_wavenet_bwd_blocks(R, d->L)) return 0;
+    uintptr_t al = reinterpret_cast<uintptr_t>(g->dx) | reinterpret_cast<uintptr_t>(a->xin) | reinterpret_cast<uintptr_t>(p->an_logs) | reinterpret_cast<uintptr_t>(p->an_bias);
+    if (g->prev_outs) {
+        if (!g->prev_xmid || (!g->prev_douts && !g->prev_douts_bf) || !g->dlogdet) return 0;
+        al |= reinterpret_cast<uintptr_t>(g->prev_xmid) | reinterpret_cast<uintptr_t>(g->prev_outs) | reinterpret_cast<uintptr_t>(g->prev_douts);
+        if (reinterpret_cast<uintptr_t>(g->prev_douts_bf) & 7) return 0;
+    }
+    return (al & 15) ? 0 : 1;
 }
 
 extern "C" int glowtts_wavenet_bwd(const glowtts_flow_dims* d, const glowtts_flow_params* p, const glowtts_flow_acts* a, const glowtts_flow_grads* g,
@@ -632,6 +781,12 @@
     const dim3 grid((unsigned)((R + nvalid - 1) / nvalid));
     hipStream_t s = static_cast<hipStream_t>(stream);
     if (cnd) { k.dcond = reinterpret_cast<float*>(g->dcond); k.ldcond = p->ldcond; }
+    if (g->fold_actnorm) {
+        if (!glowtts_wavenet_bwd_folds(d, p, a, g)) return GLOWTTS_E_ARG;
+        k.an_xin = a->xin; k.an_logs = p->an_logs; k.an_bias = p->an_bias; k.an_winfo = p->winfo; k.an_partial = g->scratch;
+        k.an_rows = g->an_rows > (int)grid.x ? g->an_rows : (int)grid.x; k.C = d->C;
+        if (g->prev_outs) { k.nc_xmid = g->prev_xmid; k.nc_outs = g->prev_outs; k.nc_douts = g->prev_douts; k.nc_douts16 = g->prev_douts_bf; k.nc_dld = g->dlogdet; }
+    }
 #ifdef GLOWTTS_TOOLS
     k.stagger = GLOWTTS_TUNABLE("GLOWTTS_WN_STAGGER", 0);
     if (!cnd && (GLOWTTS_TUNABLE("GLOWTTS_WN_BWD_ABL", 0) & 64)) k.tl = reinterpret_cast<long long*>(g->dcond);
diff --git a/glow_tts_amd/decoder.py b/glow_tts_amd/decoder.py
--- a/glow_tts_amd/decoder.py
+++ b/glow_tts_amd/decoder.py
@@ -47,7 +47,7 @@
 
 
 TAIL = {"defer": False, "pending": []}
-TUNE = {"chain_actnorm": True, "enc_ln_qkv": True, "enc_proj_ln": True, "wgrad_dma": True, "prep_fused": True, "prep_early": True, "wgrad_wide": True, "fuse_coupling_bwd": True, "act_bf16": True, "fused_wn": True, "fused_wn_bwd": -1, "fused_wn_fwd_skip": -1, "cond_hip": True, "drop_skip32": True, "wgrad_tail_splits": 2, "prep_bwd_late": False, "prep_bwd_gentle": True, "tail_aside": True, "wgrad_balance": False, "prep_twin": True}
+TUNE = {"chain_actnorm": True, "enc_ln_qkv": True, "enc_proj_ln": True, "wgrad_dma": True, "prep_fused": True, "prep_early": True, "wgrad_wide": True, "fuse_coupling_bwd": True, "act_bf16": True, "fused_wn": True, "fused_wn_bwd": -1, "fused_wn_fwd_skip": -1, "cond_hip": True, "drop_skip32": True, "wgrad_tail_splits": 2, "prep_bwd_late": False, "prep_bwd_gentle": True, "tail_aside": True, "wgrad_balance": False, "prep_twin": True, "fold_actnorm_bwd": True}
 STAMPS = {"buf": None, "names": []}
 
 
@@ -943,6 +943,7 @@
                 g.prev_xmid, g.prev_outs, g.prev_douts = buf.xmid[f - 1].data_ptr(), buf.outs[f - 1].data_ptr(), (douts[f - 1].data_ptr() if douts is not None else None)
                 g.prev_douts_bf = douts_bf[f - 1].data_ptr() if douts_bf is not None else None
             g.scratch, g.d_an, g.defer_wgrad = scratch[f].data_ptr(), None, 1
+            g.fold_actnorm, g.an_rows = int(bool(TUNE["fold_actnorm_bwd"])), nblk_all
             for l in range(Lw):
                 g.dh[l] = dh_ptr(f, l)
                 g.dins[l] = dins[f, l].data_ptr()
diff --git a/include/glowtts_hip.h b/include/glowtts_hip.h
--- a/include/glowtts_hip.h
+++ b/include/glowtts_hip.h
@@ -274,6 +274,7 @@
     float *prev_douts, *prev_douts_bf;
     const float *pitch_rows; int pitch_ns;
     int dh0_bf16;
+    int fold_actnorm, an_rows;
 } glowtts_flow_grads;
 
 int glowtts_flow_forward(const glowtts_flow_dims *d, const glowtts_flow_params *p, const glowtts_flow_acts *a, void *stream);
@@ -294,6 +295,8 @@
                         const float *xsrc, float *xdst, int reverse, int keep, void *stream);
 int glowtts_wavenet_bwd(const glowtts_flow_dims *d, const glowtts_flow_params *p, const glowtts_flow_acts *a, const glowtts_flow_grads *g,
                         void *stream);
+int glowtts_wavenet_bwd_folds(const glowtts_flow_dims *d, const glowtts_flow_params *p, const glowtts_flow_acts *a, const glowtts_flow_grads *g);
+int64_t glowtts_wavenet_bwd_blocks(int64_t rows, int L);
 
 void glowtts_wavenet_debug_safe_waits(int on);
 
```

New measurement: 5.401 million mel-frames/s. 0.982x the previous value.
